# MaaniGhaffari/cvo-rgbd

Measured on AMD Instinct MI355X. Metric: frame-pair registrations/sec, higher is better.
Workload: dtype f32; 1 GPU; BASELINE configs[1] shape: 64 distinct synthetic 10000x10000 RGB-D cloud pairs (xyz + 5-dim colour) per align_many call, cvo align() to convergence, clouds resident in HBM; points_fixed=10000, points_moving=10000, mode=cvo, batch=64

## Files before the change

### cvo-rgbd_amd/csrc/cvo_capi.cpp

```cpp
#include "cvo_internal.h"

using namespace cvo_dev;
using namespace cvo_impl;

namespace cvo_impl {

int fail(cvo_hip_ctx *ctx, int code, const char *msg)
{
    if (ctx) ctx->err = msg;
    return code;
}

static std::atomic<bool> g_engine_debug{false};
bool engine_debug_on() { return g_engine_debug.load(std::memory_order_relaxed); }

namespace {
struct OptDef {
    const char *key;
    const char *env;
    int env_kind;
    double env_value;
};
const OptDef kOptions[] = {
    {"graph_capture", "CVO_HIP_GRAPH", 1, 1.0},           {"no_graph", "CVO_HIP_NO_GRAPH", 1, 1.0},
    {"head_graphs", "CVO_HIP_RUN_GRAPHS", 1, 1.0},        {"head_mode", "CVO_HIP_NO_HEAD", 1, 0.0},
    {"resident_runs", "CVO_HIP_NO_RUN", 1, 0.0},          {"run_solvers_max", "CVO_HIP_RUN_G_MAX", 2, 0.0},
    {"run_candidates_max", "CVO_HIP_RUN_CAND", 2, 0.0},   {"run_timeout_ms", nullptr, 0, 0.0},
    {"run_fault", nullptr, 0, 0.0},                       {"merged_launches", "CVO_HIP_NO_MERGE", 1, 0.0},
    {"async_builds", "CVO_HIP_NO_ASYNC", 1, 0.0},         {"list_pass_blocks", "CVO_HIP_PROC_BLOCKS", 2, 0.0},
    {"post_debug", "CVO_HIP_POST_DEBUG", 1, 1.0},         {"mailbox_timeout_s", "CVO_HIP_MAILBOX_TIMEOUT_S", 2, 0.0},
    {"candidate_records", "CVO_HIP_NO_CAND", 1, 0.0},     {"sync_upload", "CVO_HIP_SYNC_UPLOAD", 1, 1.0},
    {"engine_debug", "CVO_HIP_ENGINE_DEBUG", 1, 1.0},     {"one_launch_hand_over", "CVO_HIP_NO_CLOUD_ONE", 1, 0.0},
    {"small_calls_alone", "CVO_HIP_NO_ALONE", 1, 0.0},    {"fused_groups", "CVO_HIP_NO_FUSE", 1, 0.0},
    {"engines", "CVO_HIP_ENGINES_FORCE", 2, 0.0},         {"list_init", "CVO_HIP_LIST_INIT", 2, 0.0},
    {"kept_pack", "CVO_HIP_NO_PACK", 1, 0.0},             {"list_margin", "CVO_HIP_LIST_MARGIN", 2, 0.0},
    {"final_mirror", "CVO_HIP_NO_FINAL_MIRROR", 1, 0.0},  {"twist_on_shared_gpu", "CVO_HIP_TWIST_ON_SHARED_GPU", 1, 1.0},
    {"comm_debug", "CVO_HIP_COMM_DEBUG", 1, 1.0},         {"wait_policy", "CVO_HIP_WAIT_POLICY", 2, 0.0},
    {"acvo_runs", "CVO_HIP_NO_ACVO_RUN", 1, 0.0},         {"tail_alone", "CVO_HIP_TAIL_ALONE", 2, 0.0},         {"side_builds", "CVO_HIP_SIDE", 1, 1.0},
    {"run_build_at", "CVO_HIP_RUN_BUILD_AT", 2, 0.0},         {"alone_max", "CVO_HIP_ALONE_MAX", 2, 0.0},
    {"narrow_merge", "CVO_HIP_NARROW_MERGE", 1, 1.0},     {"narrow_blocks", "CVO_HIP_NARROW_BLOCKS", 2, 0.0},
    {"engine_crowd", "CVO_HIP_ENGINE_CROWD", 2, 0.0},     {"engine_merge_max", "CVO_HIP_ENGINE_MERGE_MAX", 2, 0.0},
    {"matches_combine", nullptr, 0, 0.0},                 {"scan_chunk", nullptr, 0, 0.0},
    {"record_narrow", "CVO_HIP_NO_RECORD_NARROW", 1, 0.0}, {"list_stale_max", "CVO_HIP_LIST_STALE_MAX", 2, 0.0},
};
void env_defaults(cvo_hip_ctx *ctx)
{
    for (const OptDef &d : kOptions) {
        if (!d.env) continue;
        const char *e = getenv(d.env);
        if (!e) continue;
        (void)apply_option(ctx, d.key, d.env_kind == 1 ? d.env_value : atof(e));
    }
}
}

int apply_option(cvo_hip_ctx *ctx, const char *key, double v)
{
    auto is = [&](const char *k) { return std::strcmp(key, k) == 0; };
    const bool on = v != 0.0;
    CtxOptions &o = ctx->opt;
    if (is("graph_capture")) { ctx->use_graphs = on && !o.no_graph; if (!ctx->use_graphs) drop_graphs(ctx); }
    else if (is("no_graph")) { o.no_graph = on; if (on) { ctx->use_graphs = false; drop_graphs(ctx); } }
    else if (is("head_graphs")) ctx->head_graphs = on;
    else if (is("head_mode")) ctx->allow_head = on;
    else if (is("resident_runs")) ctx->allow_run = on;
    else if (is("run_solvers_max")) {
        int cus = 0;
        if (hipDeviceGetAttribute(&cus, hipDeviceAttributeMultiprocessorCount, ctx->device) != hipSuccess || cus <= 0) cus = RUN_G + 8;
        ctx->run_g_max = v > 0.0 ? std::max(8, std::min((int)RUN_G, (int)v)) : std::max(8, std::min((int)RUN_G, cus - 8));
    }
    else if (is("run_candidates_max")) { if (v < 0.0) return CVO_HIP_ERR_INVALID; o.run_cand = (int)v; }
    else if (is("run_timeout_ms")) { if (v < 0.0 || v > 6.0e4) return CVO_HIP_ERR_INVALID; o.run_timeout_ms = v; }
    else if (is("run_fault")) { if (v < 0.0) return CVO_HIP_ERR_INVALID; o.run_fault = (int)v; }
    else if (is("merged_launches")) ctx->allow_merge = on;
    else if (is("async_builds")) ctx->allow_async = ctx->allow_async_self = on;
    else if (is("list_pass_blocks")) {
        const int b = (int)v;
        if (b == 0) { ctx->proc_blocks_forced = false; ctx->proc_blocks = ctx->proc_blocks_default = PROC_BLOCKS; }
        else if (b == 64 || b == 128 || b == 256 || b == 512 || b == 1024) { ctx->proc_blocks = ctx->proc_blocks_default = b; ctx->proc_blocks_forced = true; }
        else return CVO_HIP_ERR_INVALID;
    }
    else if (is("post_debug")) o.post_debug = on;
    else if (is("mailbox_timeout_s")) { if (!(v > 0.0)) return CVO_HIP_ERR_INVALID; o.mailbox_timeout_s = v; }
    else if (is("candidate_records")) o.no_cand = !on;
    else if (is("sync_upload")) o.sync_upload = on;
    else if (is("engine_debug")) { o.engine_debug = on; if (on) g_engine_debug.store(true, std::memory_order_relaxed); }
    else if (is("one_launch_hand_over")) o.no_cloud_one = !on;
    else if (is("small_calls_alone")) o.no_alone = !on;
    else if (is("fused_groups")) o.no_fuse = !on;
    else if (is("engines")) { if (v < 0.0 || v > 8.0) return CVO_HIP_ERR_INVALID; o.engines_force = (int)v; }
    else if (is("list_init")) { if (v < 0.0) return CVO_HIP_ERR_INVALID; o.list_init = v; }
    else if (is("kept_pack")) o.no_pack = !on;
    else if (is("matches_combine")) o.matches_combine = on;
    else if (is("scan_chunk")) { if (v < 0.0 || v > (double)SCAN_CHUNK) return CVO_HIP_ERR_INVALID; o.scan_chunk = (int)v; }
    else if (is("list_margin")) { if (v > 4.0) return CVO_HIP_ERR_INVALID; o.list_margin = v < 0.0 ? -1.0f : (float)v; }
    else if (is("record_narrow")) o.record_narrow = on;
    else if (is("list_stale_max")) { if (!(v >= 1.0 && v <= 64.0)) return CVO_HIP_ERR_INVALID; o.list_stale_max = (float)v; }
    else if (is("final_mirror")) o.no_final_mirror = !on;
    else if (is("twist_on_shared_gpu")) o.twist_on_shared_gpu = on;
    else if (is("comm_debug")) o.comm_debug = on;
    else if (is("wait_policy")) { if (v < 0.0 || v > 2.0) return CVO_HIP_ERR_INVALID; o.wait_policy = (int)v; }
    else if (is("acvo_runs")) o.no_acvo_run = !on;
    else if (is("tail_alone")) { if (v < 0.0 || v > 32.0) return CVO_HIP_ERR_INVALID; o.tail_alone = (int)v; }
    else if (is("run_restart")) o.no_restart = !on;
    else if (is("side_builds")) o.no_side_builds = !on;
    else if (is("run_build_at")) { if (!(v > 0.0 && v <= 1.0)) return CVO_HIP_ERR_INVALID; o.run_build_at = (float)v; }
    else if (is("alone_max")) { if (v < 0.0 || v > 64.0) return CVO_HIP_ERR_INVALID; o.alone_max = (int)v; }
    else if (is("narrow_merge")) o.narrow_merge = on;
    else if (is("narrow_blocks")) { const int b = (int)v; if (b != 0 && b != 32 && b != 64) return CVO_HIP_ERR_INVALID; o.narrow_blocks = b; }
    else if (is("engine_crowd")) { if (v < 0.0) return CVO_HIP_ERR_INVALID; o.engine_crowd = (int)std::min(v, 1.0e6); }
    else if (is("engine_merge_max")) { if (v < 0.0 || v > 32.0) return CVO_HIP_ERR_INVALID; o.engine_merge_max = (int)v; }
    else return CVO_HIP_ERR_INVALID;
    return CVO_HIP_OK;
}

const char *params_problem(const cvo_hip_params &p)
{
    if (p.mode != CVO_HIP_MODE_CVO && p.mode != CVO_HIP_MODE_ACVO)
        return "params.mode must be CVO_HIP_MODE_CVO or CVO_HIP_MODE_ACVO (MATLAB: default_params() returns mode CVO)";
    if (p.max_iter < 0) return "params.max_iter < 0";
    const float pos[] = {p.ell_init, p.sigma, p.sp_thres, p.c, p.d, p.c_ell, p.c_sigma};
    const char *pos_name[] = {"ell_init", "sigma", "sp_thres", "c", "d", "c_ell", "c_sigma"};
    static thread_local char msg[96];
    for (int i = 0; i < 7; ++i)
        if (!(pos[i] > 0.0f) || !std::isfinite(pos[i])) {
            snprintf(msg, sizeof(msg), "params.%s must be positive and finite", pos_name[i]);
            return msg;
        }
    if (p.mode == CVO_HIP_MODE_ACVO && (!(p.c_sp_thres > 0.0f) || !std::isfinite(p.c_sp_thres)))
        return "params.c_sp_thres must be positive and finite";
    if (p.mode == CVO_HIP_MODE_ACVO && (!(p.ell_max_init > 0.0f) || !std::isfinite(p.ell_max_init) ||
                                        !(p.ell_min >= 0.0f) || !std::isfinite(p.dl_step)))
        return "params.ell_max_init / ell_min / dl_step out of range";
    const float fin[] = {p.min_step, p.eps, p.eps_2, p.color_scale, p.ell_min};
    for (float v : fin)
        if (!std::isfinite(v)) return "params: min_step, eps, eps_2, color_scale, ell_min must be finite";
    if (p.color_scale < 0.0f) return "params.color_scale < 0";
    return nullptr;
}

DevParams make_dev_params(const cvo_hip_params &p)
{
    DevParams d{};
    d.mode = p.mode;
    d.max_iter = p.max_iter;
    d.ell_init = p.ell_init;
    d.ell_min = p.ell_min;
    d.ell_max_init = p.ell_max_init;
    d.sp = p.sp_thres;
    d.c_sp = (p.mode == CVO_HIP_MODE_ACVO) ? p.c_sp_thres : p.sp_thres;
// ... 146 lines not shown
    static_assert(sizeof(DevState) >= 2048 + sizeof(DevHead), "the mirrors share a pinned DevState");
    ctx->run_mirror = ctx->done_mirror + 32;
    ctx->hint_mirror = ctx->done_mirror + 48;
    ctx->side_mirror = ctx->done_mirror + 64;
    *ctx->side_mirror = 0;
    *ctx->done_mirror = 0;
    *ctx->progress_mirror = 0;
    *ctx->run_mirror = 0;
    *ctx->hint_mirror = -1;
    {
        int cus = 0;
        if (hipDeviceGetAttribute(&cus, hipDeviceAttributeMultiprocessorCount, device) != hipSuccess || cus <= 0) cus = RUN_G + 8;
        ctx->run_g_max = std::max(8, std::min((int)RUN_G, cus - 8));
    }
    ctx->use_graphs = ctx->own_stream;
    env_defaults(ctx);
    if (ctx->opt.post_debug) {
        if (hipMalloc((void **)&ctx->post_dbg, 8 * sizeof(long long)) != hipSuccess) return bail(CVO_HIP_ERR_NOMEM);
        (void)hipMemset(ctx->post_dbg, 0, 8 * sizeof(long long));
    }
    *out = ctx;
    return CVO_HIP_OK;
}

int cvo_hip_destroy(cvo_hip_ctx *ctx)
{
    cvo_lock::Api api_guard;
    if (!ctx) return CVO_HIP_OK;
    (void)hipSetDevice(ctx->device);
    if (ctx->stream) (void)hipStreamSynchronize(ctx->stream);
    for (auto &ev : ctx->events) { (void)hipEventDestroy(ev.a); (void)hipEventDestroy(ev.b); }
    for (int i = 0; i < kPollSlots; ++i)
        if (ctx->poll_ev[i]) (void)hipEventDestroy(ctx->poll_ev[i]);
    if (ctx->comm) cvo_comm_destroy(ctx->comm);
    for (void *q : ctx->mail_opened)
        if (q) (void)hipIpcCloseMemHandle(q);
    if (ctx->comm_table) (void)hipFree(ctx->comm_table);
    if (ctx->mailbox) (void)hipFree(ctx->mailbox);
    drop_graphs(ctx);
    ctx->table.destroy();
    if (ctx->post_dbg) {
        long long h[8];
        if (hipMemcpy(h, ctx->post_dbg, sizeof(h), hipMemcpyDeviceToHost) == hipSuccess && h[0] > 0)
            fprintf(stderr, "[cvo_hip] post-step part over %lld launches, avg ticks: state load %.0f, reduce %.0f, "
                    "cubic %.0f, exp+update %.0f, prepare %.0f; head mode: block 0 of the flow launch start to end %.0f\n",
                    h[0], (double)h[1] / h[0], (double)h[2] / h[0],
                    (double)h[3] / h[0], (double)h[4] / h[0], (double)h[5] / h[0], (double)h[7] / h[0]);
        (void)hipFree(ctx->post_dbg);
    }
    for (void *p : {(void *)ctx->fixed.pos, (void *)ctx->fixed.feat, (void *)ctx->moving.pos,
                    (void *)ctx->moving.feat, (void *)ctx->fixed.seg, (void *)ctx->moving.seg,
                    (void *)ctx->scratch_a.pos, (void *)ctx->scratch_a.feat, (void *)ctx->scratch_a.seg,
                    (void *)ctx->scratch_b.pos, (void *)ctx->scratch_b.feat, (void *)ctx->scratch_b.seg, (void *)ctx->st, (void *)ctx->st2, ctx->part_flow.p, ctx->part_xx.p,
                    ctx->part_yy.p, ctx->part_step.p, ctx->part_hess.p, ctx->part_score.p, ctx->part_matches.p, ctx->run_mail.p, (void *)ctx->trace_dev, ctx->kept_cnt.p, ctx->pos_bt.p, ctx->cand[0].p, ctx->cand[1].p, ctx->cand[2].p, ctx->cand_xyb.p, ctx->cand_cnt_xyb.p, ctx->cand_sfb[0].p, ctx->cand_sfb[1].p, ctx->cand_cnt_sfb[0].p, ctx->cand_cnt_sfb[1].p, ctx->cand_cnt[0].p,
                    ctx->cand_cnt[1].p, ctx->cand_cnt[2].p})
        if (p) (void)hipFree(p);
    for (int l = 0; l < LIST_N; ++l) {
        if (ctx->lists[l].a.p) (void)hipFree(ctx->lists[l].a.p);
        if (ctx->lists[l].b.p) (void)hipFree(ctx->lists[l].b.p);
    }
    if (ctx->st_host) (void)hipHostFree(ctx->st_host);
    if (ctx->score_pin) (void)hipHostFree(ctx->score_pin);
    if (ctx->match_stage.p) (void)hipHostFree(ctx->match_stage.p);
    if (ctx->scan_stage.p) (void)hipHostFree(ctx->scan_stage.p);
    if (ctx->scan_dev.p) (void)hipFree(ctx->scan_dev.p);
    for (Cloud *c : {&ctx->fixed, &ctx->moving, &ctx->scratch_a, &ctx->scratch_b}) {
        if (c->pending && (c->wait_ev || c->ready_ev)) (void)hipEventSynchronize(c->wait_ev ? c->wait_ev : c->ready_ev);
        if (c->stage) (void)hipHostFree(c->stage);
        if (c->bbox_pin) (void)hipHostFree(c->bbox_pin);
        if (c->ready_ev) (void)hipEventDestroy(c->ready_ev);
    }
    for (DevBuf *b : {&ctx->raw_xyz, &ctx->raw_feat, &ctx->sort_keys[0], &ctx->sort_keys[1], &ctx->sort_idx[0],
                      &ctx->sort_idx[1], &ctx->sort_tmp})
        if (b->p) (void)hipFree(b->p);
    if (ctx->bbox_dev) (void)hipFree(ctx->bbox_dev);
    if (ctx->bbox_host) (void)hipHostFree(ctx->bbox_host);
    if (ctx->side_stream) { (void)hipStreamSynchronize(ctx->side_stream); (void)hipStreamDestroy(ctx->side_stream); }
    if (ctx->own_stream && ctx->stream) (void)hipStreamDestroy(ctx->stream);
    delete ctx;
    return CVO_HIP_OK;
}

int cvo_hip_set_params(cvo_hip_ctx *ctx, const cvo_hip_params *p)
{
    cvo_lock::Api api_guard;
    if (!ctx || !p) return CVO_HIP_ERR_INVALID;
    if (const char *why = params_problem(*p)) return fail(ctx, CVO_HIP_ERR_INVALID, why);
    drop_graphs(ctx);
    ctx->prm = *p;
    ctx->dprm = make_dev_params(*p);
    for (Cloud *c : {&ctx->fixed, &ctx->moving, &ctx->scratch_a, &ctx->scratch_b}) c->self.valid = false;
    return CVO_HIP_OK;
}

int cvo_hip_shard_range(int n, int rank, int world, int *lo, int *hi)
{
    if (!lo || !hi || world <= 0 || rank < 0 || rank >= world || n < 0) return CVO_HIP_ERR_INVALID;
    *lo = (int)((int64_t)n * rank / world);
    *hi = (int)((int64_t)n * (rank + 1) / world);
    return CVO_HIP_OK;
}

int cvo_hip_set_shard(cvo_hip_ctx *ctx, int row_lo, int row_hi, int srow_lo, int srow_hi)
{
    cvo_lock::Api api_guard;
    if (!ctx || row_lo < 0 || row_hi < row_lo || srow_lo < 0 || srow_hi < srow_lo)
        return CVO_HIP_ERR_INVALID;
// ... 169 lines not shown
    h->kc_ell = -1.0f;
    rc = fill_filter_geometry(ctx, h);
    if (rc) return rc;
    compute_filter_bounds(h, false);
    rc = push_state_fields(ctx, offsetof(DevState, kc),
                           offsetof(DevState, xi) - offsetof(DevState, kc));
    if (rc) return rc;
    for (bool redo = true; redo;) {
        rc = zero_counters(ctx);
        if (!rc) rc = enqueue_flow(ctx, true, 0, false, nullptr, 0);
        if (!rc) rc = check_overflow_and_grow(ctx, &redo);
        if (rc) return rc;
        if (multi_rank(ctx)) {
            double nnz = 0.0;
            rc = fetch_red(ctx, RED_FLOW + 8, 1, &nnz);
            if (rc) return rc;
            if (nnz != nnz) redo = true;
        }
    }
    rc = fetch_red(ctx, RED_FLOW, 13, out13);
    if (!rc && ctx->profiling) rc = drain_events(ctx);
    return rc;
}

int cvo_hip_step_coeffs(cvo_hip_ctx *ctx, const float omega[3], const float v[3], float ell,
                        double bcde[4])
{
    cvo_lock::Api api_guard;
    if (!ctx || !omega || !v || !bcde) return CVO_HIP_ERR_INVALID;
    HIP_TRY(ctx, hipSetDevice(ctx->device));
    if (!ctx->have_tf) return fail(ctx, CVO_HIP_ERR_INVALID, "transform_pcd not called");
    int rc = mailboxes_usable(ctx);
    if (rc) return rc;
    DevState *h = &ctx->st_host[kPollSlots];
    h->kc = make_kconsts(ctx->dprm, ell);
    h->kc_ell = -1.0f;
    rc = fill_filter_geometry(ctx, h);
    if (rc) return rc;
    compute_filter_bounds(h, false);
    h->xi = cvo_math::make_xi_consts(omega, v);
    rc = push_state_fields(ctx, offsetof(DevState, kc),
                           offsetof(DevState, omega) - offsetof(DevState, kc));
    if (rc) return rc;
    int rlo, rhi, slo, shi;
    shard_ranges(ctx, rlo, rhi, slo, shi);
    for (bool redo = true; redo;) {
        rc = zero_counters(ctx);
        if (!rc) rc = enqueue_filter(ctx, LIST_XY, ctx->fixed, rlo, rhi, 0, ctx->moving, 1, 0);
        if (!rc) rc = enqueue_process(ctx, PROC_FLOW, LIST_XY, ctx->part_flow, ctx->fixed.pos,
                                      ctx->fixed.feat, 0, ctx->moving.pos, ctx->moving.feat, 1, 0, 0);
        if (!rc) rc = check_overflow_and_grow(ctx, &redo);
        if (rc) return rc;
    }
    rc = enqueue_step(ctx, 0, false, nullptr, 0);
    if (rc) return rc;
    rc = fetch_red(ctx, RED_STEP, 4, bcde);
    if (!rc && ctx->profiling) rc = drain_events(ctx);
    return rc;
}

int cvo_hip_pick_step(const double bcde[4], float min_step, float *step)
{
    if (!bcde || !step) return CVO_HIP_ERR_INVALID;
    *step = cvo_math::pick_step(bcde, min_step);
    return CVO_HIP_OK;
}

int cvo_hip_exp_se3(const float omega[3], const float v[3], float dt, float dR[9], float dT[3])
{
    if (!omega || !v || !dR || !dT) return CVO_HIP_ERR_INVALID;
    cvo_math::exp_se3(omega, v, dt, dR, dT);
    return CVO_HIP_OK;
}

int cvo_hip_dist_se3(const float omega[3], const float v[3], float dt, float *dist)
{
    if (!omega || !v || !dist) return CVO_HIP_ERR_INVALID;
    *dist = cvo_math::dist_se3(omega, v, dt);
    return CVO_HIP_OK;
}

int cvo_hip_function_inner_product(cvo_hip_ctx *ctx, float ell, float *out)
{
    cvo_lock::Api api_guard;
    if (!ctx || !out) return CVO_HIP_ERR_INVALID;
    HIP_TRY(ctx, hipSetDevice(ctx->device));
    DevParams dp = ctx->dprm;
    dp.log_sp_s2 = (float)std::log((double)(ctx->prm.sp_thres / ctx->prm.sigma / ctx->prm.sigma));
    if (ctx->prm.mode == CVO_HIP_MODE_ACVO) {
        dp.c_sp = ctx->prm.sp_thres;
        dp.tau_c = (float)(-2.0 * ctx->prm.c_ell * ctx->prm.c_ell *
                           (double)(float)std::log((double)(dp.c_sp / ctx->prm.c_sigma / ctx->prm.c_sigma)));
    }
    int rc = mailboxes_usable(ctx);
    if (rc) return rc;
    DevState *h = &ctx->st_host[kPollSlots];
    h->kc = make_kconsts(dp, ell);
    h->kc_ell = -1.0f;
    rc = fill_filter_geometry(ctx, h);
    if (rc) return rc;
    compute_filter_bounds(h, true);
    h->done = 0;
    rc = push_state_fields(ctx, offsetof(DevState, kc),
                           offsetof(DevState, xi) - offsetof(DevState, kc));
    if (rc) return rc;
    rc = push_state_fields(ctx, offsetof(DevState, done), sizeof(int32_t));
    if (rc) return rc;
// ... 120 lines not shown
        hipMemcpy(clk, reinterpret_cast<const char *>(ctx->st) + offsetof(DevState, run_clk), sizeof(clk), hipMemcpyDeviceToHost) != hipSuccess)
        return CVO_HIP_ERR_HIP;
    for (int q = 0; q < 16; ++q) clocks16[q] = clk[q];
    return CVO_HIP_OK;
}

int cvo_hip_set_option(cvo_hip_ctx *ctx, const char *key, double value)
{
    cvo_lock::Api api_guard;
    if (!ctx || !key) return CVO_HIP_ERR_INVALID;
    if (hipSetDevice(ctx->device) != hipSuccess) return CVO_HIP_ERR_HIP;
    const int rc = apply_option(ctx, key, value);
    if (rc) return fail(ctx, rc, "cvo_hip_set_option: unknown key or value out of range");
    return CVO_HIP_OK;
}

int cvo_hip_get_option(const cvo_hip_ctx *ctx, const char *key, double *value)
{
    if (!ctx || !key || !value) return CVO_HIP_ERR_INVALID;
    auto is = [&](const char *k) { return std::strcmp(key, k) == 0; };
    const CtxOptions &o = ctx->opt;
    if (is("graph_capture")) *value = ctx->use_graphs;
    else if (is("no_graph")) *value = o.no_graph;
    else if (is("head_graphs")) *value = ctx->head_graphs;
    else if (is("head_mode")) *value = ctx->allow_head;
    else if (is("resident_runs")) *value = ctx->allow_run;
    else if (is("run_solvers_max")) *value = ctx->run_g_max;
    else if (is("run_candidates_max")) *value = o.run_cand;
    else if (is("run_timeout_ms")) *value = o.run_timeout_ms;
    else if (is("run_fault")) *value = o.run_fault;
    else if (is("merged_launches")) *value = ctx->allow_merge;
    else if (is("async_builds")) *value = ctx->allow_async;
    else if (is("list_pass_blocks")) *value = ctx->proc_blocks_forced ? ctx->proc_blocks : 0;
    else if (is("post_debug")) *value = o.post_debug;
    else if (is("mailbox_timeout_s")) *value = o.mailbox_timeout_s;
    else if (is("candidate_records")) *value = !o.no_cand;
    else if (is("sync_upload")) *value = o.sync_upload;
    else if (is("engine_debug")) *value = o.engine_debug;
    else if (is("one_launch_hand_over")) *value = !o.no_cloud_one;
    else if (is("small_calls_alone")) *value = !o.no_alone;
    else if (is("fused_groups")) *value = !o.no_fuse;
    else if (is("engines")) *value = o.engines_force;
    else if (is("narrow_merge")) *value = o.narrow_merge;
    else if (is("narrow_blocks")) *value = o.narrow_blocks;
    else if (is("engine_crowd")) *value = o.engine_crowd;
    else if (is("engine_merge_max")) *value = o.engine_merge_max;
    else if (is("list_init")) *value = o.list_init;
    else if (is("kept_pack")) *value = !o.no_pack;
    else if (is("matches_combine")) *value = o.matches_combine;
    else if (is("scan_chunk")) *value = o.scan_chunk;
    else if (is("list_margin")) *value = o.list_margin;
    else if (is("record_narrow")) *value = o.record_narrow;
    else if (is("list_stale_max")) *value = o.list_stale_max;
    else if (is("final_mirror")) *value = !o.no_final_mirror;
    else if (is("twist_on_shared_gpu")) *value = o.twist_on_shared_gpu;
    else if (is("comm_debug")) *value = o.comm_debug;
    else if (is("wait_policy")) *value = o.wait_policy;
    else if (is("acvo_runs")) *value = !o.no_acvo_run;
    else if (is("tail_alone")) *value = o.tail_alone;
    else if (is("tail_handovers")) *value = (double)ctx->tail_handovers;
    else if (is("run_restart")) *value = !o.no_restart;
    else if (is("side_builds")) *value = !o.no_side_builds;
    else if (is("run_build_at")) *value = o.run_build_at;
    else if (is("side_builds_launched")) *value = (double)ctx->side_builds_launched;
    else if (is("alone_max")) *value = o.alone_max;
    else if (is("run_timeouts")) *value = (double)ctx->run_timeouts;
    else if (is("list_grows")) *value = (double)ctx->list_grows;
    else if (is("async_builds_named")) *value = (double)ctx->async_stats[0];
    else if (is("async_stalls")) *value = (double)ctx->async_stats[1];
    else if (is("run_aborts")) *value = (double)ctx->run_aborts;
    else if (is("no_run_backoff")) *value = ctx->no_run_backoff;
    else return CVO_HIP_ERR_INVALID;
    return CVO_HIP_OK;
}

long long cvo_hip_get_mirror_retries(void) { return mirror_retries().load(std::memory_order_relaxed); }

int cvo_hip_synchronize(cvo_hip_ctx *ctx)
{
    cvo_lock::Api api_guard;
    if (!ctx) return CVO_HIP_ERR_INVALID;
    HIP_TRY(ctx, hipStreamSynchronize(ctx->stream));
    return CVO_HIP_OK;
}


}
```

### cvo-rgbd_amd/csrc/cvo_device.h

```cpp
#pragma once

#include <hip/hip_runtime.h>
#include <hip/hip_ext.h>
#include <stddef.h>
#include <stdint.h>

#include "cvo_hip.h"
#include "se3_math.hpp"

namespace cvo_dev {

constexpr int FEAT_STRIDE = 8;
constexpr int FEAT_INDEX_SLOT = 5;

constexpr int BLOCK = 256;
constexpr int TILES_PER_WAVE = 4;
constexpr int ROWS_PER_WAVE = 16 * TILES_PER_WAVE;
constexpr int ROWS_PER_TILE = 4 * ROWS_PER_WAVE;
constexpr float PAD_BIG = 1.0e30f;
constexpr int PROC_BLOCKS = 1024;
constexpr int PROC_WAVES = PROC_BLOCKS * 4;

constexpr int NSUB = 256;
constexpr int PROC_PARTS = PROC_BLOCKS / NSUB;
// ... 62 lines not shown
    unsigned long long p[RUN_GEN][RUN_CHAINS][2 * RUN_NV];
    unsigned long long entry_ticket;
    unsigned long long entry_go;
    unsigned long long side_done;
    unsigned long long side_req;
};
constexpr int RUN_G_SIDE = 128;

struct KernConsts {
    float tau;
    float tau_c;
    float sp;
    float inv_c;
    float inv_d;
    float inv_l3;
    float cb, cg, cd;
    float cscale;
    double s2_d;
    double cs2_d;
    double ninv_2l2;
    double ninv_2cl2;
};

struct DevParams {
    int32_t mode, max_iter;
    float ell_init, ell_min, ell_max_init;
    float sp, c_sp;
    float c, d, c_ell;
    float min_step, eps, eps_2;
    float log_sp_s2;
    float tau_c;
    float list_margin;
    int32_t async_xy;
    float build_at;
    int32_t async_self;
    float color_scale;
    float run_cand_cap;
    int32_t record_narrow;
    float list_stale_max;
    double s2_d, cs2_d, dl_step;
};

struct alignas(16) DevHead {
    float R[9], T[3];
    float ell, ell_max;
    float Rt[9], t[3];
    float used_Rt[9], used_t[3];
    KernConsts kc;
    float kc_ell, kc_pad_;
    float center[3];
    float xmax, y0max;
    float tauf[3];
    int32_t n_fixed;
    uint32_t pad0_;
    float list_r[3];
    int32_t list_ok[3];
    int32_t reuse[3];
    int32_t ck_nblk[3];
    float list_Rt[9], list_t[3];
    float rec_r;
    int32_t narrow;
    float rec_Rt[9], rec_t[3];
    int32_t list_stat[3];
    int32_t async_stat[2];
    int32_t rec_pad_;
    int32_t xy_active, xy_target, stall, xy_fresh;
    int32_t xy_ok[2];
    int32_t xy_ck[2];
    float xy_r[2];
    float tauf_build;
    float r_last;
    float xy_Rt[2][9], xy_t[2][3];
    int32_t sf_active[2], sf_target[2], sf_fresh[2];
    int32_t sf_ok[2][2];
    int32_t sf_ck[2][2];
    float sf_r[2][2];
    float sf_tauf_build[2];
    cvo_math::XiConsts xi;
    float omega[3], v[3];
    double dl;
    double red[RED_N];
    int32_t k;
    int32_t done;
    int32_t iter;
    int32_t n_exec;
    int32_t n_slots;
    int32_t pending;
    unsigned long long mail_snap;
    int32_t run_hint;
    int32_t head_check_;
    int32_t rec_count[2];
};
enum { REC_NARROW = 1, REC_BOUNDED = 2 };
CVO_HD unsigned head_check_mix(unsigned x, unsigned y, unsigned z, unsigned w, unsigned piece)
{
    return (x * 0x9E3779B1u + y * 0x85EBCA77u + z * 0xC2B2AE3Du + w * 0x27D4EB2Fu) ^ (piece * 0x165667B1u + 0x9E3779B9u);
}
struct DevState : DevHead {
    uint32_t sub[LIST_N][NSUB];
    uint32_t ovf[2][8];
    uint32_t built[3][64];
    int32_t run_count;
    int32_t run_entered;
    int32_t run_iterations;
    int32_t run_candidates;
    int32_t run_last_entered, run_last_aborted;
    long long run_clk[16];
    unsigned long long mail_seq;
    unsigned long long run_seq;
};
static_assert(LIST_N <= 8, "DevState::ovf holds 8 lists");
constexpr size_t DEVSTATE_INIT_BYTES = offsetof(DevState, mail_seq);
constexpr size_t DEVSTATE_HEAD_BYTES = sizeof(DevHead);
static_assert(offsetof(DevState, sub) == sizeof(DevHead) && sizeof(DevHead) % 16 == 0, "the tail follows the head");

constexpr int MAXG = 16;
template <class A> struct Grp { A a[MAXG]; };
constexpr int ENGINE_SLOTS = 32;
// ... 8 lines not shown
    TileEntry *tiles;
    TileEntry *tiles_b;
    int async_xy;
    uint32_t subcap;
    int list;
    int row_lo, row_hi;
    int nb;
    int jt;
    int tf_a, tf_b;
    int check_done;
    int gx, gy;
    long long *dbg;
    float4 *pos_bt;
};

struct ProcessArgs {
    const float4 *pos_a;
    const float *feat_a;
    const float4 *pos_b;
    const float *feat_b;
    const TileEntry *tiles;
    const TileEntry *tiles_b;
    int async_xy;
    int async_self;
    uint2 *kept_ij;
    float *kept_a;
    uint32_t *kept_cnt;
    double *partials;
    DevState *st;
    DevState *st2;
    uint32_t subcap;
    uint32_t kept_wcap;
    int nblk;
    const double *flow_part;
    const double *xx_part;
    const double *yy_part;
    cvo_hip_trace *trace; int trace_cap;
    int acvo;
    int32_t *done_mirror;
    int list;
    int row_hi, nb;
    int first_counted;
    int tf_a, tf_b;
    int check_done;
    int weight;
    uint2 *cand;
    uint32_t *cand_cnt;
    uint2 *cand_b;
    uint32_t *cand_cnt_b;
    int need_d2;
    const CommTable *comm;
    int kept_packed;
    unsigned kept_ebase;
};

enum { POST_REDUCE = 1, POST_MATH = 2 };

struct PostFlowArgs {
    DevState *st;
    const double *part_flow;
    const double *part_xx;
    const double *part_yy;
    cvo_hip_trace *trace; int trace_cap;
    int flags;
    int check_done;
    int32_t *done_mirror;
    int nblk;
    const CommTable *comm;
    DevParams prm;
};

struct PostStepArgs {
    DevState *st;
    DevState *st2;
    const double *part_step;
    cvo_hip_trace *trace; int trace_cap;
    int flags;
    int check_done;
    long long *dbg;
    int32_t *done_mirror;
    int ck_nblk[3];
    int32_t *progress_mirror;
    int nblk;
    const CommTable *comm;
    DevHead *final_mirror;
    uint32_t *build_mask;
    uint32_t slot_bit;
    RunMail *run_mail;
    int32_t *run_mirror;
    int32_t *hint_mirror;
    int run_iters;
    int run_g_max;
    long long run_timeout_ticks;
    int32_t *side_mirror;
    float run_build_at;
    int run_fault;
    DevParams prm;
};

constexpr size_t kTableHeaderBytes = 256;
constexpr int MAX_OPS = 10;
struct OpArgs {
    ProcessArgs p;
    FilterArgs f;
    union {
        PostFlowArgs pf;
        PostStepArgs ps;
    };
    int np, n0, n1, n2;
};
struct Slot {
    int active;
    int pad_[3];
    OpArgs op[MAX_OPS];
};

CVO_HD KernConsts make_kconsts(const DevParams &p, float ell)
{
    KernConsts k;
    const float l = ell;
    k.tau = (float)(-2.0 * l * l * (double)p.log_sp_s2);
    k.tau_c = p.tau_c;
    k.sp = p.sp;
// ... 604 lines not shown
```

### cvo-rgbd_amd/csrc/cvo_internal.h

```cpp
#pragma once
#include "cvo_hip.h"

#include <hip/hip_runtime.h>

#include <algorithm>
#include <atomic>
#include <chrono>
#include <cmath>
#include <cstddef>
#include <cstdint>
#include <cstdio>
#include <cstdlib>
#include <cstring>
#include <deque>
#include <memory>
#include <mutex>
#include <new>
#include <string>
#include <thread>
#include <vector>

#include "cvo_cloud.h"
#include "cvo_comm.h"
#include "cvo_device.h"
// ... 119 lines not shown
            st[z] = image[(size_t)z];
        }
        if (hipMemcpyAsync(&dev[lo], &st[lo], n * sizeof(Slot), hipMemcpyHostToDevice, s) != hipSuccess) return -1;
        if (arm(s) != 0) return -1;
        if (hipEventRecord(stage_ev[b], s) != hipSuccess) return -1;
        stage_used[b] = true;
        return 0;
    }
};

struct PlanGraph {
    std::vector<TLaunch> pre;
    std::vector<TLaunch> plan;
    int iterations = 0;
    hipGraph_t graph = nullptr;
    hipGraphExec_t exec = nullptr;
    uint64_t stamp = 0;
};
struct PlanCache {
    std::vector<PlanGraph> graphs;
    uint64_t clock = 0;
    long long hits = 0, captures = 0;
    int fails = 0;
    void drop()
    {
        for (auto &g : graphs) {
            if (g.exec) (void)hipGraphExecDestroy(g.exec);
            if (g.graph) (void)hipGraphDestroy(g.graph);
        }
        graphs.clear();
    }
};
constexpr int kPollSlots = 4;
constexpr int kEvProcFlow = 10, kEvProcStep = 11;
constexpr int kProcStepTwist = 100;
constexpr int kFlowBuild = 101;
constexpr int kFilterAhead = 102;

struct RecOp {
    enum Kind { FILTER, PROCESS, POST_FLOW, POST_STEP } kind;
    int mode = 0;
    FilterArgs f{};
    ProcessArgs p{};
    PostFlowArgs pf{};
    PostStepArgs ps{};
};


}

using namespace cvo_dev;
using namespace cvo_impl;

struct CtxOptions {
    bool no_cand = false;
    bool no_graph = false;
    bool sync_upload = false;
    bool engine_debug = false;
    bool no_cloud_one = false;
    bool no_alone = false;
    bool no_fuse = false;
    bool no_pack = false;
    bool matches_combine = true;
    int scan_chunk = 0;
    bool no_final_mirror = false;
    bool twist_on_shared_gpu = false;
    bool comm_debug = false;
    bool post_debug = false;
    bool no_side_builds = true;
    float run_build_at = 0.6f;
    bool no_restart = false;
    bool no_acvo_run = false;
    int tail_alone = 8;
    int alone_max = 0;
    int engines_force = 0;
    int narrow_blocks = 0;
    bool narrow_merge = false;
    int engine_crowd = 2;
    int engine_merge_max = 2;
    double list_init = 0.0;
    float list_margin = -1.0f;
    bool record_narrow = true;
    float list_stale_max = 3.0f;
    int run_cand = 0;
    double mailbox_timeout_s = 5.0;
    double run_timeout_ms = 0.0;
    int run_fault = 0;
    int wait_policy = 0;
};

struct cvo_hip_ctx {
    CtxOptions opt;
    int no_run_backoff = 0;
    long long side_builds_launched = 0;
    long long tail_handovers = 0;
    long long run_aborts = 0;
    int list_stats[3] = {0, 0, 0};
    int async_stats[2] = {0, 0};
    long long list_grows = 0;
    long long run_timeouts = 0;
    int device = 0;
    hipStream_t stream = nullptr;
    bool own_stream = false;
    cvo_hip_params prm{};
    DevParams dprm{};
    Cloud fixed, moving;
    Cloud scratch_a, scratch_b;
    DevState *st = nullptr;
    DevHead *st2 = nullptr;
    bool head_mode = false;
    bool allow_head = true;
    DevState *st_host = nullptr;
    int32_t *done_mirror = nullptr;
    int32_t *progress_mirror = nullptr;
    DevHead *final_mirror = nullptr;
    int32_t *run_mirror = nullptr;
    int32_t *hint_mirror = nullptr;
    int32_t *side_mirror = nullptr;
    hipStream_t side_stream = nullptr;
    std::vector<TLaunch> plan_side;
    DevBuf run_mail;
    bool plan_has_final_mirror = false;
    bool allow_run = true;
    int run_g_max = RUN_G;
    int run_g_call = RUN_G;
    bool call_no_spec = false;
    int big_run_backoff = 0;
    bool spec_first_run = true;
    bool head_graphs = false;
    int run_small_max = 0;
    int run_nnz_max = 0;
    std::vector<TLaunch> plan_pre;
    std::vector<RecOp> *rec = nullptr;
    int proc_blocks = PROC_BLOCKS;
    int proc_blocks_default = PROC_BLOCKS;
    bool proc_blocks_forced = false;
    DevBuf raw_xyz, raw_feat;
    DevBuf sort_keys[2], sort_idx[2], sort_tmp;
    float *bbox_dev = nullptr;
    float *bbox_host = nullptr;
    FilterArgs xy_build{};
    bool have_xy_build = false;
    bool allow_async = true;
    bool crowded = false;
    DevBuf cand[3], cand_cnt[3];
    DevBuf cand_xyb, cand_cnt_xyb;
    DevBuf cand_sfb[2], cand_cnt_sfb[2];
    int ck_nblk[3] = {0, 0, 0};
    DevBuf pos_bt;
    bool lone = true;
    bool allow_async_self = true;
    bool use_async_self = false;
    bool use_async = false;
    bool in_loop = false;
    bool plan_recording = false;
    bool merge_twist = false;
    bool allow_merge = true;
    cvo_hip_trace *cur_trace = nullptr;
    int cur_trace_cap = 0;
    hipEvent_t poll_ev[kPollSlots]{};
    DevBuf part_flow, part_xx, part_yy, part_step;
    DevBuf part_hess;
    DevBuf part_score;
    struct ScorePin *score_pin = nullptr;
    DevBuf part_matches;
    PinBuf match_stage;
    DevBuf scan_dev;
    PinBuf scan_stage;
    List lists[LIST_N];
    DevBuf kept_cnt;
    cvo_hip_trace *trace_dev = nullptr;
    int trace_dev_cap = 0;
    bool have_tf = false;
    int row_lo = 0, row_hi = -1, srow_lo = 0, srow_hi = -1;
    bool sharded = false;
    cvo_comm *comm = nullptr;
    Mailbox *mailbox = nullptr;
    CommTable *comm_table = nullptr;
    void *mail_opened[MAX_WORLD] = {};
    int mail_rank = 0, mail_world = 0;
    bool mail_shared_device = false;
    unsigned long long mail_dev_id = 0;
    bool mail_broken = false;
    cvo_hip_allreduce_fn user_allreduce = nullptr;
    void *user_allreduce_arg = nullptr;
    bool profiling = false;
    long long *post_dbg = nullptr;
    TableBuf table;
    PlanCache plans;
    std::vector<TLaunch> plan;
    hipStream_t loop_stream = nullptr;
    bool warm = false;
    bool use_graphs = true;
    int iter_tag = -1;
    std::vector<EventPair> events;
    cvo_hip_profile prof{};
    std::string err;
};

namespace cvo_impl {

// ... 12 lines not shown
    cvo_hip_trace *trace = nullptr;
    int trace_cap = 0;
    int *n_iter = nullptr;
    int enq = 0;
    int batches = 0;
    int checked = 0;
    int executed_base = 0;
    int phase = 0;
    int rc = CVO_HIP_OK;
    bool in_group = false;
    int runs_enq = 0;
    bool run_waiting = false;
    bool spec_pending = false;
    bool paced_nb = false;
    int idle_seen = 0;
    int side_seen = 0;
    int side_launched = 0;
    int restarts = 0;
    bool paced = false;
};

int fail(cvo_hip_ctx *ctx, int code, const char *msg);
bool engine_debug_on();
int apply_option(cvo_hip_ctx *ctx, const char *key, double value);
inline bool runs_allowed(const cvo_hip_ctx *ctx) { return ctx->allow_run && ctx->no_run_backoff <= 0; }
const char *params_problem(const cvo_hip_params &p);
DevParams make_dev_params(const cvo_hip_params &p);
int cloud_ready(cvo_hip_ctx *ctx, Cloud &c);
int cloud_reserve(cvo_hip_ctx *ctx, Cloud &c, const float *xyz, const float *feat, int n, int layout);
int upload_cloud(cvo_hip_ctx *ctx, Cloud &c, const float *xyz, const float *feat, int n, int layout, bool on_device = false);
FilterPlan plan_filter(int nrows, int nb);
int ensure_buf(cvo_hip_ctx *ctx, DevBuf &b, size_t bytes);
int ensure_list(cvo_hip_ctx *ctx, int list, int nrows, int nb, double at_least);
void shard_ranges(const cvo_hip_ctx *ctx, int &rlo, int &rhi, int &slo, int &shi);
int fill_filter_geometry(cvo_hip_ctx *ctx, DevState *h);
int mailboxes_usable(cvo_hip_ctx *ctx);
bool host_reduce(const cvo_hip_ctx *ctx);
bool multi_rank(const cvo_hip_ctx *ctx);
DevParams loop_params(const cvo_hip_ctx *ctx);
hipStream_t loop_stream(const cvo_hip_ctx *ctx);
int enqueue_filter(cvo_hip_ctx *ctx, int list, const Cloud &ca, int row_lo, int row_hi, int tf_a, const Cloud &cb, int tf_b, int check_done);
int kept_format(const cvo_hip_ctx *ctx, unsigned *ebase);
KeptView kept_view(const cvo_hip_ctx *ctx);
int enqueue_process(cvo_hip_ctx *ctx, int mode, int list, DevBuf &part, const float4 *pos_a, const float *feat_a, int tf_a,
                    const float4 *pos_b, const float *feat_b, int tf_b, int first_counted, int check_done);
int drain_events(cvo_hip_ctx *ctx, int n_exec = -1, const DevState *fin = nullptr);
int reduce_over_ranks(cvo_hip_ctx *ctx, int off, int count);
int enqueue_flow(cvo_hip_ctx *ctx, bool tf_moving, int check_done, bool do_math, cvo_hip_trace *trace, int trace_cap);
int enqueue_step(cvo_hip_ctx *ctx, int check_done, bool do_math, cvo_hip_trace *trace, int trace_cap);
int check_overflow_and_grow(cvo_hip_ctx *ctx, bool *redo);
int prepare_buffers(cvo_hip_ctx *ctx);
int enqueue_iterations(cvo_hip_ctx *ctx, int count, int tag0, int trace_cap);
void drop_graphs(cvo_hip_ctx *ctx);
TLaunch mk_launch(int kernel, int q, unsigned gx, unsigned gz, unsigned smem = 0);
bool plan_lone(const std::vector<RecOp> &ops, Slot &slot, std::vector<TLaunch> &plan, const bool allow_head, bool *head_mode,
               std::vector<TLaunch> *pre = nullptr, std::vector<TLaunch> *side = nullptr);
void set_build_masks(Slot &slot, const std::vector<TLaunch> &plan, uint32_t *masks, int z);
bool plan_fused(const std::vector<const std::vector<RecOp> *> &ops, const std::vector<Slot *> &slots, int zdim, std::vector<TLaunch> &plan);
int run_plan(const Slot *tab, PlanCache &cache, const std::vector<TLaunch> &plan, hipStream_t s, bool use_graph, int iterations,
             const std::vector<TLaunch> *pre = nullptr);
int record_iteration(cvo_hip_ctx *ctx, std::vector<RecOp> &ops, int trace_cap);
int prepare_lone_plan(cvo_hip_ctx *ctx, int trace_cap);
int launch_batch(cvo_hip_ctx *ctx, int tag0, int trace_cap, bool with_run = false, int slots = kBatch, bool small_run = false, bool two_runs = false);
constexpr int kNoRunBackoff = 64;
constexpr int kBigRunBackoff = 16;
constexpr int kShortBatch = 2;
constexpr int kRunBatchSlots = 2;
int zero_counters(cvo_hip_ctx *ctx);
int push_state_fields(cvo_hip_ctx *ctx, size_t off, size_t bytes);
int push_pose_fields(cvo_hip_ctx *ctx, const DevHead *img, bool with_consts);
int enqueue_flow_reduce(cvo_hip_ctx *ctx, const CommTable *comm);
int fetch_red(cvo_hip_ctx *ctx, int off, int count, double *out);
void decide_scheme(cvo_hip_ctx *ctx);
std::atomic<long long> &mirror_retries();
int job_begin(AlignJob &j);
int job_finish(AlignJob &j);
int job_continue_alone(AlignJob &j);
int job_pump(AlignJob &j, bool block);

}
```

### cvo-rgbd_amd/csrc/cvo_job.cpp

```cpp
#include "cvo_internal.h"

using namespace cvo_dev;
using namespace cvo_impl;

namespace cvo_impl {

void decide_scheme(cvo_hip_ctx *ctx)
{
    const bool small_pair = (double)ctx->fixed.n * (double)ctx->moving.n <= 2.5e7;
    if (!ctx->proc_blocks_forced)
        ctx->proc_blocks = ctx->proc_blocks_default = small_pair ? PROC_BLOCKS / 2 : PROC_BLOCKS;
    ctx->use_async = ctx->allow_async && !ctx->crowded && !ctx->profiling && !multi_rank(ctx) &&
                     !(ctx->prm.color_scale > 0.0f) &&
                     (double)ctx->fixed.n * (double)ctx->moving.n <= 2.0e8;
    ctx->use_async_self = ctx->use_async && ctx->allow_async_self && ctx->lone &&
                          ctx->prm.mode == CVO_HIP_MODE_ACVO;
    const double npairs = (double)ctx->fixed.n * (double)ctx->moving.n;
    if (ctx->use_async_self && !ctx->proc_blocks_forced)
        ctx->proc_blocks = ctx->proc_blocks_default = npairs <= 6.0e7 ? PROC_BLOCKS / 8 : PROC_BLOCKS / 4;
    if (!ctx->proc_blocks_forced && !ctx->use_async_self && ctx->use_async && ctx->lone && ctx->allow_head &&
        ctx->prm.mode == CVO_HIP_MODE_CVO)
    {
        const bool runs = runs_allowed(ctx) && ctx->fixed.np <= 65536 && ctx->moving.np <= 65536;
        ctx->proc_blocks = ctx->proc_blocks_default =
// ... 110 lines not shown
    decide_scheme(ctx);
    hipStream_t s = loop_stream(ctx);
    HIP_TRY(ctx, hipMemsetAsync(reinterpret_cast<char *>(ctx->st) + offsetof(DevState, n_slots), 0, sizeof(int32_t), s));
    HIP_TRY(ctx, hipMemsetAsync(reinterpret_cast<char *>(ctx->st) + offsetof(DevState, run_count), 0, 4 * sizeof(int32_t), s));
    HIP_TRY(ctx, hipMemsetAsync(reinterpret_cast<char *>(ctx->st) + offsetof(DevState, run_last_entered), 0, 2 * sizeof(int32_t), s));
    launch_prepare(ctx->st, loop_params(ctx), s, ctx->table.raw ? ctx->table.masks() : nullptr);
    HIP_TRY(ctx, hipGetLastError());
    const int prc = prepare_buffers(ctx);
    if (prc) return prc;
    ctx->head_mode = false;
    const int rc = prepare_lone_plan(ctx, 0);
    if (rc) return rc;
    j.enq = j.batches = j.checked = 0;
    j.runs_enq = 0;
    j.run_waiting = false;
    j.spec_pending = false;
    j.side_seen = 0;
    j.side_launched = 0;
    const int g_call = std::max(8, std::min(ctx->run_g_max, ctx->run_g_call));
    ctx->run_nnz_max = g_call * RUN_BLOCK * (RUN_R + RUN_L);
    ctx->run_small_max = 3 * RUN_G_SMALL * RUN_BLOCK;
    if (ctx->prm.mode == CVO_HIP_MODE_ACVO) {
        ctx->run_nnz_max = (int)(0.8 * g_call * RUN_BLOCK * RUN_A);
        ctx->run_small_max = (int)(0.8 * 2 * RUN_G_SMALL * RUN_BLOCK);
    }
    if (ctx->opt.run_cand > 0) ctx->run_nnz_max = ctx->opt.run_cand;
    j.phase = 0;
    ++ctx->tail_handovers;
    return CVO_HIP_OK;
}

int job_finish(AlignJob &j)
{
    cvo_hip_ctx *ctx = j.ctx;
    cvo_hip_state *s = j.s;
    const DevState &f = ctx->st_host[0];
    ctx->have_tf = false;
    if (f.done == DONE_COMM_ERROR) {
        ctx->mail_broken = true;
        if (ctx->opt.comm_debug)
            fprintf(stderr, "[cvo_hip] rank %d of %d: exchange timed out at iteration k = %d (executed %d), mail_seq %llu, mail_snap %llu, slots %d, twist in launch %d\n",
                    ctx->mail_rank, ctx->mail_world, f.k, f.n_exec, (unsigned long long)f.mail_seq, (unsigned long long)f.mail_snap, f.n_slots,
                    (int)(ctx->plan.size() == 4));
        return fail(ctx, CVO_HIP_ERR_COMM, "mailbox all-reduce timed out: a peer rank never delivered its partial sums "
                                           "(the mailboxes must be created and connected again on every rank)");
    }
    if (f.done == DONE_RUN_TIMEOUT)
        return fail(ctx, CVO_HIP_ERR_RUN, "a resident run timed out and the registration could not be redone without runs");
    if (f.done == RUNNING || f.done == NEED_BIGGER_LIST)
        return fail(ctx, CVO_HIP_ERR_INVALID, "align loop ended without a verdict");
    const int executed = f.n_exec;
    for (int q = 0; q < 3; ++q) ctx->list_stats[q] = f.list_stat[q];
    for (int q = 0; q < 2; ++q) ctx->async_stats[q] = f.async_stat[q];
    if (j.trace_cap > 0 && executed > 0)
        HIP_TRY(ctx, hipMemcpy(j.trace, ctx->trace_dev,
                               (size_t)std::min(executed, j.trace_cap) * sizeof(cvo_hip_trace),
                               hipMemcpyDeviceToHost));
    if (executed > 0) cvo_math::tf_to_mat4(f.used_Rt, f.used_t, s->transform);
    std::memcpy(s->R, f.R, sizeof(s->R));
    std::memcpy(s->T, f.T, sizeof(s->T));
    s->ell = f.ell;
    s->ell_max = f.ell_max;
    s->iter = f.iter;
    std::memcpy(s->prev_transform, s->transform, sizeof(s->transform));
    cvo_math::mat4_mul(s->accum_transform, s->transform, s->accum_transform);
    float Rt[9], t[3];
    cvo_math::inverse_tf(s->R, s->T, Rt, t);
    cvo_math::tf_to_mat4(Rt, t, s->transform);
    if (j.n_iter) *j.n_iter = executed;
    if (ctx->profiling) return drain_events(ctx, executed, &f);
    return CVO_HIP_OK;
}

int job_pump(AlignJob &j, bool block)
{
    cvo_hip_ctx *ctx = j.ctx;
    if (j.phase == 2) return 1;
    auto finish_with = [&](int rc) { j.rc = rc; j.phase = 2; return 1; };
    if (hipSetDevice(ctx->device) != hipSuccess) return finish_with(CVO_HIP_ERR_HIP);
    if (j.phase == 0 && (block || j.paced_nb) && (j.paced || j.paced_nb) && !host_reduce(ctx) && !ctx->profiling) {
        const int limit = (ctx->use_async ? 3 : 1) * ctx->prm.max_iter + 4 * kBatch;
        unsigned spins = 0;
        int idle_seen = 0;
        const auto t_enter = std::chrono::steady_clock::now();
        for (;;) {
            if (*(volatile int32_t *)ctx->done_mirror != RUNNING) break;
            const int runs_word = *(volatile int32_t *)ctx->run_mirror;
            const int runs = runs_word & (RUN_MIRROR_ABORTED - 1);
            const int slots = *(volatile int32_t *)ctx->progress_mirror;
            if (!ctx->plan_side.empty()) {
                const int want = *(volatile int32_t *)ctx->side_mirror;
                if (want != 0 && want != j.side_seen) {
                    j.side_seen = want;
                    for (const TLaunch &l : ctx->plan_side) launch_table(ctx->table.dev, l, ctx->side_stream);
                    if (hipGetLastError() != hipSuccess) return finish_with(fail(ctx, CVO_HIP_ERR_HIP, "launching a side build failed"));
                    ++j.side_launched;
                    ++ctx->side_builds_launched;
                }
            }
            const int lead = ctx->head_mode ? 2 : 0;
            bool go;
            if (j.run_waiting) {
                go = runs >= j.runs_enq;
                if (go) {
                    if (runs_word & RUN_MIRROR_ABORTED) { ctx->big_run_backoff = kBigRunBackoff; ++ctx->run_aborts; }
                    else if (j.spec_pending) ctx->spec_first_run = (runs_word & RUN_MIRROR_ENTERED) != 0;
// ... 216 lines not shown
```

### cvo-rgbd_amd/csrc/cvo_kernels.hip

```cpp
#include <algorithm>
#include <atomic>
#include <cstdlib>

#include "cvo_device.h"
#include "cvo_pair.h"

namespace cvo_dev {

typedef float f32x4 __attribute__((ext_vector_type(4)));

__device__ __forceinline__ float mv_row(const float *m, float x, float y, float z)
{
    return (m[0] * x + m[1] * y) + m[2] * z;
}

constexpr int FILTER_KMAX = 64;
size_t filter_smem_bytes(int jt)
{
    return (size_t)jt * 16 + ROWS_PER_TILE * 16 + 4 * TILE_STAGE * sizeof(TileEntry) +
           FILTER_KMAX * 4 * 4;
}

__device__ __forceinline__ void flush_tiles(const TileEntry *stage, int n, int lane, unsigned rot, unsigned region,
                                            const FilterArgs &a, int list, TileEntry *tiles, const int par)
{
    static_assert(TILE_STAGE <= 128, "two entries per lane");
    constexpr int sh = DEAL_SHIFT, L = 1 << sh;
    unsigned base = 0;
    if (lane < 32) {
        int cnt = 0;
        for (int c = (int)(((unsigned)lane - rot) & 31u); (c << sh) < n; c += 32) cnt += min(n - (c << sh), L);
        if (cnt) base = atomicAdd(&a.st->sub[list][((unsigned)lane << 3) | region], (unsigned)cnt);
    }
    bool over = false;
#pragma unroll
    for (int h = 0; h < 2; ++h) {
        const int k = lane + 64 * h;
        const unsigned c = (unsigned)k >> sh;
        const unsigned j = (c + rot) & 31u;
        const unsigned pos = (unsigned)__shfl((int)base, (int)j, 64) + ((c >> 5) << sh) + ((unsigned)k & (unsigned)(L - 1));
        if (k < n) {
            if (pos < a.subcap) tiles[(size_t)((j << 3) | region) * a.subcap + pos] = stage[k];
            else over = true;
        }
    }
    if (__ballot(over) != 0ull && lane == 0)
        atomicOr(&a.st->ovf[par][list], 1u);
}

__device__ __forceinline__ void pretransform_body(const FilterArgs &a, const unsigned bid, const unsigned nblocks)
{
    if (!a.pos_bt) return;
    if (a.check_done && a.st->done != 0) return;
    const float *Rt = a.st->Rt;
    const float *tt = a.st->t;
    for (unsigned j = bid * BLOCK + threadIdx.x; j < (unsigned)a.nb; j += nblocks * BLOCK) {
        const float4 y0 = a.pos_b[j];
        float4 y = apply_tf(Rt, tt, y0);
        y.w = y0.w;
        a.pos_bt[j] = y;
    }
}

template <bool PIPE = true>
__device__ __forceinline__ void filter_body(const FilterArgs &a, const unsigned bid, const unsigned nblocks,
                                            const DevState *__restrict__ hd, const int par)
{
// ... 226 lines not shown
    const long long want = std::min<long long>(per_region * 8, std::max<long long>(cap, 8));
    return (unsigned)((want + 7) / 8 * 8);
}

void launch_filter(const FilterArgs &a, dim3 grid, hipStream_t s, hipEvent_t ev_start,
                   hipEvent_t ev_stop)
{
    Grp<FilterArgs> g;
    g.a[0] = a;
    g.a[0].gx = (int)grid.x; g.a[0].gy = (int)grid.y;
    grid = dim3(filter_grid_x((long long)grid.x * grid.y, filter_blocks_max()), 1, 1);
    if (ev_start && ev_stop)
        hipExtLaunchKernelGGL(k_filter, grid, dim3(BLOCK), filter_smem_bytes(a.jt), s, ev_start,
                              ev_stop, 0, g);
    else
        hipLaunchKernelGGL(k_filter, grid, dim3(BLOCK), filter_smem_bytes(a.jt), s, g);
}

void launch_filter_group(const FilterArgs *a, int n, hipStream_t s)
{
    Grp<FilterArgs> g;
    dim3 grid(1, 1, (unsigned)n);
    int jt = 0;
    const long long cap = std::max<long long>(64, filter_blocks_max() / (2 * n));
    for (int i = 0; i < n; ++i) {
        g.a[i] = a[i];
        grid.x = std::max(grid.x, filter_grid_x((long long)a[i].gx * a[i].gy, cap));
        jt = std::max(jt, a[i].jt);
    }
    hipLaunchKernelGGL(k_filter, grid, dim3(BLOCK), filter_smem_bytes(jt), s, g);
}


__device__ __forceinline__ float colour_weight(const KernConsts &kc, const float4 fa0, const float fa4,
                                               const float4 fb0, const float fb4, const double *etab)
{
    const float d2c = d2_feat(fa0, fa4, fb0, fb4);
    if (!(d2c < kc.tau_c)) return 0.0f;
    return (float)(kc.cs2_d * exp_neg((double)d2c * kc.ninv_2cl2, etab));
}
__device__ __forceinline__ float weight_from_ck(const KernConsts &kc, float d2, float ck, const double *etab)
{
    const float k = (float)(kc.s2_d * exp_neg((double)d2 * kc.ninv_2l2, etab));
    const float a = ck * k;
    return a > kc.sp ? a : 0.0f;
}


template <int MODE> struct NAcc;
template <> struct NAcc<PROC_FLOW> { static constexpr int n = NACC_FLOW; };
template <> struct NAcc<PROC_STEP> { static constexpr int n = NACC_STEP; };
template <> struct NAcc<PROC_SELF> { static constexpr int n = NACC_SELF; };

__device__ __forceinline__ double div6(double x)
{
    const double c = 0x1.5555555555555p-3;
    const double q0 = x * c;
    const double r = __builtin_fma(-6.0, q0, x);
    return __builtin_fma(r, c, q0);
}

__device__ __forceinline__ uint2 list_load(const uint2 *p)
{
#ifdef CVO_NT_LISTS
    typedef unsigned u32x2 __attribute__((ext_vector_type(2)));
    const u32x2 v = __builtin_nontemporal_load(reinterpret_cast<const u32x2 *>(p));
    return make_uint2(v.x, v.y);
#else
    return *p;
#endif
}

__device__ __forceinline__ const float4 *gather16(const void *base, unsigned byte_off)
{
    return reinterpret_cast<const float4 *>(static_cast<const char *>(base) + byte_off);
}

struct ProcHead {
    const float *Rt, *tt;
    const cvo_math::XiConsts *xi;
    KernConsts kc;
    int done_word;
    int n_fixed;
    int second;
    unsigned list_bad;
    int ck_nblk;
    int par;
    uint2 *cand;
    uint32_t *cand_cnt;
    int need_d2;
    int narrow;
    float rec_lim;
};

template <int MODE>
__device__ __forceinline__ ProcHead proc_head_global(const ProcessArgs &a, const DevState *st, const int par)
{
    ProcHead h;
    h.Rt = st->Rt; h.tt = st->t; h.xi = &st->xi;
    h.kc = st->kc;
    h.done_word = a.check_done ? (st->done | (a.async_xy ? st->stall : 0)) : 0;
    h.n_fixed = (MODE == PROC_SELF && a.first_counted) ? st->n_fixed : 0;
    h.second = ((MODE == PROC_FLOW && a.async_xy && st->xy_active == 1) ||
                (MODE == PROC_SELF && a.async_self && st->sf_active[a.async_self - 1] == 1)) ? 1 : 0;
    const bool ahead = (MODE == PROC_FLOW && a.async_xy) || (MODE == PROC_SELF && a.async_self);
    h.list_bad = ahead ? 0u : a.st->ovf[par][MODE == PROC_STEP ? (int)LIST_KEPT : a.list];
    h.ck_nblk = st->ck_nblk[a.list];
    h.par = par;
    h.cand = a.cand; h.cand_cnt = a.cand_cnt;
    h.need_d2 = a.need_d2;
    h.narrow = (MODE == PROC_FLOW && !a.async_xy) ? st->narrow : 0;
    h.rec_lim = (h.narrow & REC_BOUNDED) ? st->rec_r * st->rec_r : PAD_BIG;
    return h;
}


struct PairSrc {
    const CVO_GLOBAL char *pos_a; const float *feat_a;
    const CVO_GLOBAL char *pos_b; const float *feat_b;
    int tf_a, tf_b;
};
#ifdef CVO_NO_PIN
constexpr bool kPinBuild = false;
#else
constexpr bool kPinBuild = true;
#endif
#ifdef CVO_NO_PF
constexpr bool kPrefetchBuild = false;
#else
constexpr bool kPrefetchBuild = true;
#endif
template <bool PIN, class T> __device__ __forceinline__ const CVO_GLOBAL char *pin_global(const T *p)
{
    unsigned long long v = (unsigned long long)p;
    if (PIN && kPinBuild) asm volatile("" : "+s"(v));
    return (const CVO_GLOBAL char *)v;
}
template <bool PIN> __device__ __forceinline__ unsigned pin_u32(unsigned v)
{
    if (PIN && kPinBuild) asm volatile("" : "+s"(v));
    return v;
}
template <bool PIN> __device__ __forceinline__ PairSrc pin_pair_src(const ProcessArgs &a)
{
    PairSrc p;
    p.pos_a = pin_global<PIN>(a.pos_a); p.pos_b = pin_global<PIN>(a.pos_b);
    p.feat_a = a.feat_a; p.feat_b = a.feat_b;
    p.tf_a = (int)pin_u32<PIN>((unsigned)a.tf_a); p.tf_b = (int)pin_u32<PIN>((unsigned)a.tf_b);
    return p;
}
__device__ __forceinline__ void store8(const CVO_GLOBAL char *base, unsigned idx, unsigned x, unsigned y)
{
    u32x2_t v; v.x = x; v.y = y;
    CVO_GLOBAL u32x2_t *q = reinterpret_cast<CVO_GLOBAL u32x2_t *>(const_cast<CVO_GLOBAL char *>(base)) + idx;
#ifdef CVO_NT_KEPT_ST
    __builtin_nontemporal_store(v, q);
#else
    *q = v;
#endif
}

__device__ __forceinline__ cvo_math::XiConsts xi_uniform(const cvo_math::XiConsts &g)
{
    cvo_math::XiConsts xc;
    auto uni = [](float x) { return __int_as_float(__builtin_amdgcn_readfirstlane(__float_as_int(x))); };
#pragma unroll
    for (int q = 0; q < 3; ++q) {
        xc.omega[q] = uni(g.omega[q]); xc.v[q] = uni(g.v[q]);
        xc.u2[q] = uni(g.u2[q]); xc.u3[q] = uni(g.u3[q]); xc.u4[q] = uni(g.u4[q]);
    }
#pragma unroll
    for (int q = 0; q < 9; ++q) {
        xc.W2[q] = uni(g.W2[q]); xc.W3[q] = uni(g.W3[q]); xc.W4[q] = uni(g.W4[q]);
    }
    return xc;
}

__device__ __forceinline__ void pair_flow_sums(const KernConsts &kc, const float4 xi, const float4 yj, const float w, const float d2,
                                           const int need_d2, double *acc)
{
    const float c0 = xi.y * yj.z - xi.z * yj.y;
    const float c1 = xi.z * yj.x - xi.x * yj.z;
    const float c2 = xi.x * yj.y - xi.y * yj.x;
    const float f0 = yj.x - xi.x, f1 = yj.y - xi.y, f2 = yj.z - xi.z;
    const float ac = kc.inv_c * w, ad = kc.inv_d * w;
    acc[0] += (double)(ac * c0);
    acc[1] += (double)(ac * c1);
    acc[2] += (double)(ac * c2);
    acc[3] += (double)(ad * f0);
    acc[4] += (double)(ad * f1);
    acc[5] += (double)(ad * f2);
#ifdef CVO_SUM_A_ALWAYS
    acc[6] += (double)w;
    if (need_d2) acc[7] += (double)((kc.inv_l3 * w) * d2);
#else
    if (need_d2) {
        acc[6] += (double)w;
        acc[7] += (double)((kc.inv_l3 * w) * d2);
    }
#endif
}

__device__ __forceinline__ void step_tail(const float w, const float beta, const float gamma, const float delta, const float epsil, double *acc)
{
    const double A = (double)w;
    const double b = (double)beta, g = (double)gamma;
    acc[0] += (double)(w * beta);
#ifdef CVO_STEP_TAIL_LITERAL
    acc[1] += A * (g + (double)(beta * beta) / 2.0);
    acc[2] += A * ((double)(delta + beta * gamma) + div6((double)(beta * beta * beta)));
    acc[3] += A * ((((double)(epsil + beta * delta) + 0.5 * b * b * g) + 0.5 * g * g) +
                   1 / 24.0 * b * b * b * b);
#else
    acc[1] = __builtin_fma(A, __builtin_fma((double)(beta * beta), 0.5, g), acc[1]);
    acc[2] = __builtin_fma(A, __builtin_fma((double)(beta * beta * beta), 0x1.5555555555555p-3,
                                            (double)(delta + beta * gamma)), acc[2]);
    const double b2 = b * b, hg = 0.5 * g;
    double t = __builtin_fma(b2, hg, (double)(epsil + beta * delta));
    t = __builtin_fma(hg, g, t);
    t = __builtin_fma(b2 * (1 / 24.0), b2, t);
    acc[3] = __builtin_fma(A, t, acc[3]);
#endif
}

__device__ __forceinline__ void pair_step_sums(const KernConsts &kc, const cvo_math::XiConsts &xc, const float4 yj, const float e0,
                                           const float e1, const float e2, const float w, double *acc)
{
    float xiz[3], xi2z[3], xi3z[3], xi4z[3];
    xiz[0] = (xc.omega[1] * yj.z - xc.omega[2] * yj.y) + xc.v[0];
    xiz[1] = (xc.omega[2] * yj.x - xc.omega[0] * yj.z) + xc.v[1];
    xiz[2] = (xc.omega[0] * yj.y - xc.omega[1] * yj.x) + xc.v[2];
#pragma unroll
    for (int r = 0; r < 3; ++r) {
        xi2z[r] = mv_row(xc.W2 + 3 * r, yj.x, yj.y, yj.z) + xc.u2[r];
        xi3z[r] = mv_row(xc.W3 + 3 * r, yj.x, yj.y, yj.z) + xc.u3[r];
        xi4z[r] = mv_row(xc.W4 + 3 * r, yj.x, yj.y, yj.z) + xc.u4[r];
    }
    const float normxiz2 = (xiz[0] * xiz[0] + xiz[1] * xiz[1]) + xiz[2] * xiz[2];
    const float xz12 = -((xiz[0] * xi2z[0] + xiz[1] * xi2z[1]) + xiz[2] * xi2z[2]);
    const float eps_c = ((xi2z[0] * xi2z[0] + xi2z[1] * xi2z[1]) + xi2z[2] * xi2z[2]) +
                        2 * ((xiz[0] * xi3z[0] + xiz[1] * xi3z[1]) + xiz[2] * xi3z[2]);
    const float cb = kc.cb, cg = kc.cg, cd = kc.cd;
    const float beta = ((cb * xiz[0]) * e0 + (cb * xiz[1]) * e1) + (cb * xiz[2]) * e2;
    const float g_dot = ((2.0f * xi2z[0]) * e0 + (2.0f * xi2z[1]) * e1) + (2.0f * xi2z[2]) * e2;
    const float gamma = cg * (normxiz2 + g_dot);
    const float d_dot = ((-xi3z[0]) * e0 + (-xi3z[1]) * e1) + (-xi3z[2]) * e2;
    const float delta = cd * (xz12 + d_dot);
    const float e_dot = ((2.0f * xi4z[0]) * e0 + (2.0f * xi4z[1]) * e1) + (2.0f * xi4z[2]) * e2;
    const float epsil = cg * (eps_c + e_dot);
    step_tail(w, beta, gamma, delta, epsil, acc);
}

typedef float f32x2 __attribute__((ext_vector_type(2)));
__device__ __forceinline__ void pair_step_sums2(const KernConsts &kc, const cvo_math::XiConsts &xc, const f32x2 yx, const f32x2 yy, const f32x2 yz,
                                                const f32x2 e0, const f32x2 e1, const f32x2 e2, const f32x2 w, double *acc)
{
    f32x2 xiz[3], xi2z[3], xi3z[3], xi4z[3];
    xiz[0] = (xc.omega[1] * yz - xc.omega[2] * yy) + xc.v[0];
    xiz[1] = (xc.omega[2] * yx - xc.omega[0] * yz) + xc.v[1];
    xiz[2] = (xc.omega[0] * yy - xc.omega[1] * yx) + xc.v[2];
#pragma unroll
    for (int r = 0; r < 3; ++r) {
        xi2z[r] = ((xc.W2[3 * r] * yx + xc.W2[3 * r + 1] * yy) + xc.W2[3 * r + 2] * yz) + xc.u2[r];
        xi3z[r] = ((xc.W3[3 * r] * yx + xc.W3[3 * r + 1] * yy) + xc.W3[3 * r + 2] * yz) + xc.u3[r];
        xi4z[r] = ((xc.W4[3 * r] * yx + xc.W4[3 * r + 1] * yy) + xc.W4[3 * r + 2] * yz) + xc.u4[r];
    }
    const f32x2 normxiz2 = (xiz[0] * xiz[0] + xiz[1] * xiz[1]) + xiz[2] * xiz[2];
    const f32x2 xz12 = -((xiz[0] * xi2z[0] + xiz[1] * xi2z[1]) + xiz[2] * xi2z[2]);
    const f32x2 eps_c = ((xi2z[0] * xi2z[0] + xi2z[1] * xi2z[1]) + xi2z[2] * xi2z[2]) +
                        2.0f * ((xiz[0] * xi3z[0] + xiz[1] * xi3z[1]) + xiz[2] * xi3z[2]);
    const float cb = kc.cb, cg = kc.cg, cd = kc.cd;
    const f32x2 beta = ((cb * xiz[0]) * e0 + (cb * xiz[1]) * e1) + (cb * xiz[2]) * e2;
    const f32x2 g_dot = ((2.0f * xi2z[0]) * e0 + (2.0f * xi2z[1]) * e1) + (2.0f * xi2z[2]) * e2;
    const f32x2 gamma = cg * (normxiz2 + g_dot);
    const f32x2 d_dot = ((-xi3z[0]) * e0 + (-xi3z[1]) * e1) + (-xi3z[2]) * e2;
    const f32x2 delta = cd * (xz12 + d_dot);
    const f32x2 e_dot = ((2.0f * xi4z[0]) * e0 + (2.0f * xi4z[1]) * e1) + (2.0f * xi4z[2]) * e2;
    const f32x2 epsil = cg * (eps_c + e_dot);
    step_tail(w.x, beta.x, gamma.x, delta.x, epsil.x, acc);
    step_tail(w.y, beta.y, gamma.y, delta.y, epsil.y, acc);
}

template <int MODE, int WEIGHT = 0, int CK = 0, class ARGS = ProcessArgs>
__device__ __forceinline__ float eval_pair(const ARGS &a, const ProcHead &hd, const KernConsts &kc, unsigned i,
                                           unsigned j, float w, double *acc,
                                           const cvo_math::XiConsts &xc, const double *etab = nullptr,
                                           const int first_counted = 0, float *ck_io = nullptr,
                                           uint2 *pf_out = nullptr, const CVO_GLOBAL char *pf_base = nullptr, unsigned pf_idx = 0,
                                           float *d2_out = nullptr )
{
    const float *Rt = hd.Rt;
    const float *tt = hd.tt;
    constexpr bool need_w = MODE != PROC_STEP && CK != 2;
    float4 xi = load_pos<need_w>(a.pos_a, i * 16u);
    float4 yj = load_pos<need_w>(a.pos_b, j * 16u);
    if (pf_out) *pf_out = load8(pf_base, pf_idx);
    float4 fa0 = make_float4(0.f, 0.f, 0.f, 0.f), fb0 = fa0;
    float fa4 = 0.f, fb4 = 0.f;
    int row_index = 0;
    if (MODE != PROC_STEP && CK != 2) {
        fa0 = *gather16(a.feat_a, i * (unsigned)(FEAT_STRIDE * 4));
        fb0 = *gather16(a.feat_b, j * (unsigned)(FEAT_STRIDE * 4));
// ... 23 lines not shown
        pair_flow_sums(kc, xi, yj, w, d2, hd.need_d2, acc);
    } else if (MODE == PROC_STEP) {
#ifdef CVO_PROBE_STEP_EXP
        {
            const float d2p = __builtin_fmaf(e2, e2, __builtin_fmaf(e1, e1, e0 * e0));
            const float kp = (float)(kc.s2_d * exp_neg((double)d2p * kc.ninv_2l2, etab ? etab : c_exp2_64));
            asm volatile("" ::"v"(kp));
        }
#endif
        pair_step_sums(kc, xc, yj, e0, e1, e2, w, acc);
    } else {
        if (CK == 2 ? row_index >= 0 : row_index >= first_counted) acc[0] += (double)((kc.inv_l3 * w) * d2);
    }
    return w;
}

template <bool PF>
__device__ __forceinline__ void step_members2(const PairSrc &src, const ProcHead &hd, const KernConsts &kc, const cvo_math::XiConsts &xc,
                                              const CVO_GLOBAL char *kept_w, const float *kept_a, const int packed, const unsigned ebase,
                                              const unsigned wcap, const unsigned n, const int lane, uint2 e, float w, double *acc)
{
    const float *Rt = hd.Rt, *tt = hd.tt;
    uint2 eb = load8(kept_w, min((unsigned)lane + 64u, wcap - 1u));
    for (unsigned off = lane; off < n; off += 128u) {
        const bool two = off + 64u < n;
        if (off >= 128u && !PF) { e = load8(kept_w, off); eb = load8(kept_w, min(off + 64u, wcap - 1u)); }
        float wa = w, wb = 0.0f;
        if (!packed) { wa = kept_a[off]; wb = kept_a[min(off + 64u, wcap - 1u)]; }
        if (!two) { eb = e; wb = wa; }
        unsigned ia, ja, ib, jb;
        float ma, mb;
        kept_unpack(packed, ebase, e, wa, ia, ja, ma);
        kept_unpack(packed, ebase, eb, wb, ib, jb, mb);
        if (!two) mb = 0.0f;
        const float4 xa = load_pos<false>(src.pos_a, ia * 16u), ya = load_pos<false>(src.pos_b, ja * 16u);
        const float4 xb = load_pos<false>(src.pos_a, ib * 16u), yb = load_pos<false>(src.pos_b, jb * 16u);
        if (PF) { e = load8(kept_w, min(off + 128u, wcap - 1u)); eb = load8(kept_w, min(off + 192u, wcap - 1u)); }
        f32x2 px = {xa.x, xb.x}, py = {xa.y, xb.y}, pz = {xa.z, xb.z};
        f32x2 qx = {ya.x, yb.x}, qy = {ya.y, yb.y}, qz = {ya.z, yb.z};
        if (src.tf_a) {
            const f32x2 ox = ((Rt[0] * px + Rt[1] * py) + Rt[2] * pz) + tt[0];
            const f32x2 oy = ((Rt[3] * px + Rt[4] * py) + Rt[5] * pz) + tt[1];
            const f32x2 oz = ((Rt[6] * px + Rt[7] * py) + Rt[8] * pz) + tt[2];
            px = ox; py = oy; pz = oz;
        }
        if (src.tf_b) {
            const f32x2 ox = ((Rt[0] * qx + Rt[1] * qy) + Rt[2] * qz) + tt[0];
            const f32x2 oy = ((Rt[3] * qx + Rt[4] * qy) + Rt[5] * qz) + tt[1];
            const f32x2 oz = ((Rt[6] * qx + Rt[7] * qy) + Rt[8] * qz) + tt[2];
            qx = ox; qy = oy; qz = oz;
        }
        const f32x2 mw = {ma, mb};
        pair_step_sums2(kc, xc, qx, qy, qz, px - qx, py - qy, pz - qz, mw, acc);
    }
}

constexpr int PROC_SMEM = 4 * NACC_MAX * 8 + 4 * PAIR_QUEUE * 8 + 4 * 64 * 8;

template <int MODE, int WEIGHT, int REC, bool PIPE>
__device__ __forceinline__ bool expand_lists(const ProcessArgs &a, const ProcHead &hd, const KernConsts &kc, const unsigned bid, const int wid,
                                             const int lane, const unsigned wave, const int done_word,
                                             const unsigned list_bad, const int in_list, const TileEntry *in_tiles,
                                             const int first_counted, const double *s_etab, uint2 *pairq_all,
                                             double (&acc)[NAcc<MODE>::n])
{
        const bool shared = a.nblk >= NSUB;
        const unsigned nsl = shared ? 1u : (unsigned)(NSUB / a.nblk);
        const unsigned part = shared ? bid / NSUB : 0u;
        unsigned sub = bid & (NSUB - 1);
        unsigned n = list_bad ? 0u : a.st->sub[in_list][sub];
        const TileEntry *tl = in_tiles + (size_t)sub * a.subcap;
        const unsigned stride = shared ? 4u * (unsigned)(a.nblk / NSUB) : 4u;
        const unsigned e0 = part * 4u + (unsigned)wid;
        TileEntry mine = tl[min(e0 + (unsigned)lane * stride, a.subcap - 1)];
        if (done_word != 0) return false;
        uint2 *pairq = pairq_all + wid * PAIR_QUEUE;
        const PairSrc src = pin_pair_src<PIPE>(a);
        int qn = 0;
        unsigned nk = 0;
        unsigned co = 0;
        const size_t kbase = (size_t)wave * a.kept_wcap;
        auto run_batch = [&](int base, int cnt) {
            __builtin_amdgcn_fence(__ATOMIC_RELEASE, "wavefront");
            __builtin_amdgcn_wave_barrier();
            __builtin_amdgcn_fence(__ATOMIC_ACQUIRE, "wavefront");
            float w = 0.0f;
            uint2 pr = make_uint2(0u, 0u);
            float ck = 0.0f;
            float d2 = 0.0f;
            if (lane < cnt) {
                pr = pairq[base + lane];
                w = eval_pair<MODE, WEIGHT, REC>(src, hd, kc, pr.x, pr.y, 0.0f, acc, *hd.xi, s_etab, first_counted, &ck,
                                                 nullptr, nullptr, 0, (REC && MODE == PROC_FLOW) ? &d2 : nullptr);
            }
            if (REC && MODE == PROC_FLOW) {
                const unsigned long long cm = __ballot(lane < cnt && !(d2 >= hd.rec_lim));
                const unsigned add = (unsigned)__popcll(cm);
                if (co + add <= a.kept_wcap) {
                    if (lane < cnt && !(d2 >= hd.rec_lim)) {
                        const unsigned below = __builtin_amdgcn_mbcnt_hi((unsigned)(cm >> 32), __builtin_amdgcn_mbcnt_lo((unsigned)cm, 0u));
                        hd.cand[kbase + co + below] = make_uint2(pr.x | (pr.y << 16), __float_as_uint(ck));
                    }
                } else if (lane == 0) {
                    atomicOr(&a.st->ovf[hd.par][LIST_KEPT], 1u);
                }
                co += add;
// ... 140 lines not shown
        acc[MODE == PROC_FLOW ? 8 : 1] = (double)nk;
        if (NARROW) hd.cand_cnt[wave] = co;
    }
    return true;
}

template <int MODE, int WEIGHT = 0, bool CAND = true, bool PIPE = true>
__device__ __forceinline__ void process_body(const ProcessArgs &a, const unsigned bid, char *scratch, const ProcHead &hd)
{
    if ((int)bid >= a.nblk) return;
    constexpr int NACC = NAcc<MODE>::n;
    double *red = reinterpret_cast<double *>(scratch);
    uint2 *pairq_all = reinterpret_cast<uint2 *>(scratch + 4 * NACC_MAX * 8);
    double *s_etab_all = reinterpret_cast<double *>(scratch + 4 * NACC_MAX * 8 + 4 * PAIR_QUEUE * 8);
#ifdef CVO_PROBE_STEP_EXP
    s_etab_all[threadIdx.x] = c_exp2_64[threadIdx.x & 63];
#else
    if (MODE != PROC_STEP) s_etab_all[threadIdx.x] = c_exp2_64[threadIdx.x & 63];
#endif
    const double *s_etab = s_etab_all + ((MODE == PROC_STEP) ? 0 : (threadIdx.x >> 6) * 64);
    const int tid = threadIdx.x, lane = tid & 63;
    const int wid = __builtin_amdgcn_readfirstlane(tid >> 6);
    const unsigned wave = bid * 4u + (unsigned)wid;
    const int done_word = hd.done_word;
    const KernConsts kc = hd.kc;
    const int first_counted = hd.n_fixed;
    const bool second = hd.second != 0;
    const int in_list = !second ? a.list : (MODE == PROC_FLOW ? (int)LIST_XYB : self_list_id(a.async_self - 1, 1));
    const TileEntry *in_tiles = second ? a.tiles_b : a.tiles;
    const unsigned list_bad = hd.list_bad;

    double acc[NACC];
#pragma unroll
    for (int k = 0; k < NACC; ++k) acc[k] = 0.0;

    if (MODE == PROC_STEP) {
        const size_t base = (size_t)wave * a.kept_wcap;
        unsigned n = a.kept_cnt[wave];
        const int packed = a.kept_packed;
        uint2 e = list_load(&a.kept_ij[base + lane]);
        float w = packed ? 0.0f : a.kept_a[base + lane];
        if (done_word != 0) return;
        if (n > a.kept_wcap) n = a.kept_wcap;
        if (list_bad) n = 0;
        const PairSrc src = pin_pair_src<PIPE>(a);
        const cvo_math::XiConsts xc = xi_uniform(*hd.xi);
        const CVO_GLOBAL char *kept_w = pin_global<PIPE>(a.kept_ij + base);
        const unsigned ebase = pin_u32<PIPE>(a.kept_ebase), wcap = pin_u32<PIPE>(a.kept_wcap);
        constexpr bool PF = PIPE && kPrefetchBuild;
#if defined(CVO_STEP_TWO) && !defined(CVO_PROBE_STEP_EXP)
        step_members2<PF>(src, hd, kc, xc, kept_w, a.kept_a + base, packed, ebase, wcap, n, lane, e, w, acc);
        if (false)
#endif
        for (unsigned off = lane; off < n; off += 64) {
            if (off >= 64) { if (!PF) e = load8(kept_w, off); if (!packed) w = a.kept_a[base + off]; }
            uint2 e_next = e;
            uint2 *const pf = PF ? &e_next : nullptr;
            unsigned mi, mj;
            float mw;
            kept_unpack(packed, ebase, e, w, mi, mj, mw);
#ifdef CVO_PROBE_STEP_EXP
            eval_pair<MODE>(src, hd, kc, mi, mj, mw, acc, xc, s_etab, 0, nullptr, pf, kept_w, min(off + 64u, wcap - 1u));
#else
            eval_pair<MODE>(src, hd, kc, mi, mj, mw, acc, xc, nullptr, 0, nullptr, pf, kept_w, min(off + 64u, wcap - 1u));
#endif
            if (PF) e = e_next;
        }
    } else {
        bool alive;
        if (CAND && WEIGHT == 0 && hd.cand && (MODE == PROC_FLOW ? (!a.async_xy || a.cand_b != nullptr)
                                                                 : (!a.async_self || a.cand_b != nullptr))) {
            if (hd.ck_nblk == a.nblk && MODE == PROC_FLOW && (hd.narrow & REC_NARROW))
                alive = stream_candidates<MODE, PIPE, MODE == PROC_FLOW>(a, hd, kc, lane, wave, done_word, s_etab, acc);
            else if (hd.ck_nblk == a.nblk) alive = stream_candidates<MODE, PIPE>(a, hd, kc, lane, wave, done_word, s_etab, acc);
            else alive = expand_lists<MODE, WEIGHT, WEIGHT == 0 ? 1 : 0, PIPE>(a, hd, kc, bid, wid, lane, wave, done_word, list_bad, in_list, in_tiles, first_counted, s_etab, pairq_all, acc);
        } else {
            alive = expand_lists<MODE, WEIGHT, 0, PIPE>(a, hd, kc, bid, wid, lane, wave, done_word, list_bad, in_list, in_tiles, first_counted, s_etab, pairq_all, acc);
        }
        if (!alive) return;
    }

    wave_sums<NACC>(acc, lane, red + wid * NACC);
    __syncthreads();
    if (tid < NACC) {
        const double s = ((red[tid] + red[NACC + tid]) + red[2 * NACC + tid]) + red[3 * NACC + tid];
        a.partials[(size_t)tid * a.nblk + bid] = s;
    }
}

template <int MODE, int WEIGHT = 0>
__global__ void __launch_bounds__(BLOCK) k_process(const Grp<ProcessArgs> grp)
{
    __shared__ __attribute__((aligned(16))) char scratch[PROC_SMEM];
    const ProcessArgs &a = grp.a[blockIdx.z];
    process_body<MODE, WEIGHT>(a, blockIdx.x, scratch, proc_head_global<MODE>(a, a.st, 0));
}

constexpr int STEP_BLOCK = 1024;
constexpr int STEP_WAVES = STEP_BLOCK / 64;

__device__ __forceinline__ void xi_consts_wave(cvo_math::XiConsts *xi, float *wm, const float omega[3], const float v[3], const int lane)
{
    if (lane == 0) {
        const cvo_math::Mat3 W = cvo_math::skew(omega);
#pragma unroll
        for (int k = 0; k < 9; ++k) wm[k] = W.m[k];
// ... 97 lines not shown
    const bool overflow = s_overflow != 0;
    if (blockIdx.x == 0 && tid == 0) {
        DevState *st = hd;
        if (overflow) {
            st->done = NEED_BIGGER_LIST;
            if (a.done_mirror) *a.done_mirror = NEED_BIGGER_LIST;
        } else {
            for (int q = 0; q < NACC_FLOW; ++q) st->red[RED_FLOW + q] = tot[q];
            for (int q = 0; q < 4; ++q) st->red[RED_XX + q] = a.acvo ? tot[NACC_FLOW + q] : 0.0;
            for (int q = 0; q < 3; ++q) { st->omega[q] = s_xi.omega[q]; st->v[q] = s_xi.v[q]; }
            st->xi = s_xi;
            double dl = 0.0;
            const long long nnz = (long long)tot[8];
            long long nnz_xx = 0, nnz_yy = 0;
            if (a.acvo) {
                nnz_xx = (long long)tot[NACC_FLOW + 1];
                nnz_yy = (long long)tot[NACC_FLOW + 3];
                const double num = (tot[NACC_FLOW + 2] - 2.0 * tot[7]) + tot[NACC_FLOW];
                dl = num / (double)(nnz_xx + nnz_yy - 2 * nnz);
            }
            st->dl = dl;
            if (a.trace && st->k < a.trace_cap) {
                cvo_hip_trace &tr = a.trace[st->k];
                tr.k = st->k;
                tr.exit_code = 0;
                tr.ell = st->ell;
                for (int q = 0; q < 3; ++q) {
                    tr.omega[q] = s_xi.omega[q]; tr.v[q] = s_xi.v[q];
                    tr.omega_d[q] = tot[q]; tr.v_d[q] = tot[3 + q];
                }
                tr.sum_a = tot[6];
                tr.dl = dl;
                tr.nnz = nnz; tr.nnz_xx = nnz_xx; tr.nnz_yy = nnz_yy;
            }
        }
    }
    if (overflow) return false;
    cvo_math::XiConsts xc;
    {
        auto uni = [](float x) { return __int_as_float(__builtin_amdgcn_readfirstlane(__float_as_int(x))); };
#pragma unroll
        for (int q = 0; q < 3; ++q) {
            xc.omega[q] = uni(s_xi.omega[q]); xc.v[q] = uni(s_xi.v[q]);
            xc.u2[q] = uni(s_xi.u2[q]); xc.u3[q] = uni(s_xi.u3[q]); xc.u4[q] = uni(s_xi.u4[q]);
        }
#pragma unroll
        for (int q = 0; q < 9; ++q) {
            xc.W2[q] = uni(s_xi.W2[q]); xc.W3[q] = uni(s_xi.W3[q]); xc.W4[q] = uni(s_xi.W4[q]);
        }
    }

    ProcHead phd;
    phd.need_d2 = 0;
    phd.narrow = 0; phd.rec_lim = PAD_BIG;
    phd.Rt = hd->Rt; phd.tt = hd->t;
    double acc[NACC];
#pragma unroll
    for (int k = 0; k < NACC; ++k) acc[k] = 0.0;
    unsigned wcap = a.kept_wcap, ebase = a.kept_ebase;
    if (n > wcap) n = wcap;
    const PairSrc src = pin_pair_src<true>(a);
    const CVO_GLOBAL char *kept_w = pin_global<true>(a.kept_ij + base);
    wcap = pin_u32<true>(wcap); ebase = pin_u32<true>(ebase);
    constexpr bool PF = kPrefetchBuild;
    for (unsigned off = lane; off < n; off += 64) {
        if (off >= 64) { if (!PF) e = load8(kept_w, off); if (!packed) w = a.kept_a[base + off]; }
        uint2 e_next = e;
        uint2 *const pf = PF ? &e_next : nullptr;
        unsigned mi, mj;
        float mw;
        kept_unpack(packed, ebase, e, w, mi, mj, mw);
        eval_pair<PROC_STEP>(src, phd, kc, mi, mj, mw, acc, xc, nullptr, 0, nullptr, pf, kept_w, min(off + 64u, wcap - 1u));
        if (PF) e = e_next;
    }
    __syncthreads();
    wave_sums<NACC>(acc, lane, sh + wid * NACC);
    __syncthreads();
    if (tid < NACC) {
        double t = 0.0;
#pragma unroll
        for (int q = 0; q < STEP_WAVES; ++q) t += sh[q * NACC + tid];
        a.partials[(size_t)tid * nfat + blockIdx.x] = t;
    }
    return true;
}

__global__ void __launch_bounds__(STEP_BLOCK) k_step_twist(const Grp<ProcessArgs> grp)
{
    step_twist_body(grp.a[blockIdx.z], grp.a[blockIdx.z].st, 0, false);
}

void launch_step_twist_group(const ProcessArgs *a, int n, hipStream_t s, hipEvent_t ev_start, hipEvent_t ev_stop)
{
    Grp<ProcessArgs> g;
    int nblk = 32;
    for (int i = 0; i < n; ++i) { g.a[i] = a[i]; nblk = std::max(nblk, a[i].nblk); }
    const dim3 grid((unsigned)(nblk / (STEP_BLOCK / BLOCK)), 1, (unsigned)n);
    if (ev_start && ev_stop) hipExtLaunchKernelGGL(k_step_twist, grid, dim3(STEP_BLOCK), 0, s, ev_start, ev_stop, 0, g);
    else hipLaunchKernelGGL(k_step_twist, grid, dim3(STEP_BLOCK), 0, s, g);
}

void launch_process_group(int mode, const ProcessArgs *a, int n, hipStream_t s, hipEvent_t ev_start, hipEvent_t ev_stop)
{
    Grp<ProcessArgs> g;
    for (int i = 0; i < n; ++i) g.a[i] = a[i];
    int nblk = 1;
    for (int i = 0; i < n; ++i) nblk = std::max(nblk, a[i].nblk);
// ... 156 lines not shown
            *sh_fail = all_ok ? 0 : 1;
        }
    }
    __syncthreads();
    return *sh_fail == 0;
}

__device__ bool mailbox_allreduce_every_block(const CommTable &ct, DevState *gst, const DevHead *hd, double *vals, int count,
                                              double *sh , int *sh_fail)
{
    __syncthreads();
    const int lane = threadIdx.x;
    if (lane < 64) {
        const unsigned long long seq = hd->mail_snap + 1ull;
        const int gen = (int)(seq & 1ull);
        bool ok = true;
        if (lane < ct.world) {
            if (blockIdx.x == 0) {
                MailSlot *dst = &ct.peer[lane]->slot[gen][ct.rank];
                for (int i = 0; i < count; ++i)
                    __hip_atomic_store(&dst->v[i], vals[i], __ATOMIC_RELAXED, __HIP_MEMORY_SCOPE_SYSTEM);
                __builtin_amdgcn_fence(__ATOMIC_RELEASE, "");
                asm volatile("s_waitcnt vmcnt(0)" ::: "memory");
                __hip_atomic_store(&dst->seq, seq, __ATOMIC_RELAXED, __HIP_MEMORY_SCOPE_SYSTEM);
            }
            const MailSlot *src = &ct.peer[ct.rank]->slot[gen][lane];
            const long long t0 = (long long)wall_clock64();
            while (__hip_atomic_load(&src->seq, __ATOMIC_RELAXED, __HIP_MEMORY_SCOPE_SYSTEM) != seq) {
                if ((long long)wall_clock64() - t0 > ct.timeout_ticks) { ok = false; break; }
                __builtin_amdgcn_s_sleep(8);
            }
            __builtin_amdgcn_fence(__ATOMIC_ACQUIRE, "");
            for (int i = 0; i < count; ++i)
                sh[lane * MAIL_VALS + i] = __hip_atomic_load(&src->v[i], __ATOMIC_RELAXED, __HIP_MEMORY_SCOPE_SYSTEM);
        }
        const bool all_ok = __ballot(!ok) == 0ull;
        __builtin_amdgcn_fence(__ATOMIC_RELEASE, "wavefront");
        __builtin_amdgcn_wave_barrier();
        __builtin_amdgcn_fence(__ATOMIC_ACQUIRE, "wavefront");
        if (lane < count && all_ok) {
            double t = 0.0;
            for (int r = 0; r < ct.world; ++r) t += sh[r * MAIL_VALS + lane];
            vals[lane] = t;
        }
        if (lane == 0) {
            if (blockIdx.x == 0) gst->mail_seq = seq;
            *sh_fail = all_ok ? 0 : 1;
        }
    }
    __syncthreads();
    return *sh_fail == 0;
}

__device__ __forceinline__ void post_flow_body(const PostFlowArgs &a)
{
    __shared__ double sh[4 * NACC_MAX];
    __shared__ __attribute__((aligned(16))) DevHead s_st;
    state_head_to_lds(a.st, &s_st);
    DevHead *st = &s_st;
    if (a.check_done && (st->done != 0 || (a.prm.async_xy && st->stall))) return;
    const bool acvo = a.prm.mode == CVO_HIP_MODE_ACVO;
    if (a.flags & POST_REDUCE) {
        block_reduce_partials<NACC_FLOW>(a.part_flow, a.nblk, sh, st->red + RED_FLOW);
        if (acvo) {
            block_reduce_partials<NACC_SELF>(a.part_xx, a.nblk, sh, st->red + RED_XX);
            block_reduce_partials<NACC_SELF>(a.part_yy, a.nblk, sh, st->red + RED_YY);
        } else if (threadIdx.x == 0) {
            st->red[RED_XX] = st->red[RED_XX + 1] = st->red[RED_YY] = st->red[RED_YY + 1] = 0.0;
        }
        if (threadIdx.x == 0 &&
            ((a.prm.async_xy ? 0u : a.st->ovf[0][LIST_XY]) | a.st->ovf[0][LIST_XX] |
             a.st->ovf[0][LIST_YY] | a.st->ovf[0][LIST_KEPT]))
            st->red[8] = __builtin_nan("");
    }
    bool comm_ok = true;
    if (a.comm) {
        __shared__ double sh_mail[MAX_WORLD * MAIL_VALS];
        __shared__ int sh_fail;
        comm_ok = mailbox_allreduce(*a.comm, a.st, st->red + RED_FLOW, RED_STEP - RED_FLOW, sh_mail, &sh_fail, st);
        if (!comm_ok && threadIdx.x == 0) st->done = DONE_COMM_ERROR;
    }
    if ((a.flags & POST_MATH) && comm_ok && threadIdx.x < 64) {
        const double *red = st->red;
        float omega[3], v[3];
        for (int q = 0; q < 3; ++q) { omega[q] = (float)red[q]; v[q] = (float)red[3 + q]; }
        if (!(red[8] != red[8])) xi_consts_wave(&st->xi, reinterpret_cast<float *>(sh), omega, v, (int)threadIdx.x);
    }
    if ((a.flags & POST_MATH) && comm_ok && threadIdx.x == 0) {
        const bool overflow = st->red[8] != st->red[8];
        if (overflow) st->done = NEED_BIGGER_LIST;
        const double *red = st->red;
        float omega[3], v[3];
        for (int q = 0; q < 3; ++q) {
            omega[q] = (float)red[q];
            v[q] = (float)red[3 + q];
            st->omega[q] = omega[q];
            st->v[q] = v[q];
        }
        double dl = 0.0;
        const long long nnz = (long long)red[8];
        long long nnz_xx = 0, nnz_yy = 0;
        if (acvo) {
            nnz_xx = (long long)red[RED_XX + 1];
            nnz_yy = (long long)red[RED_YY + 1];
            const double num = (red[RED_YY] - 2.0 * red[7]) + red[RED_XX];
            dl = num / (double)(nnz_xx + nnz_yy - 2 * nnz);
        }
        st->dl = dl;
        if (!overflow && a.trace && st->k < a.trace_cap) {
            cvo_hip_trace &tr = a.trace[st->k];
            tr.k = st->k;
            tr.exit_code = 0;
            tr.ell = st->ell;
            for (int q = 0; q < 3; ++q) {
                tr.omega[q] = omega[q]; tr.v[q] = v[q];
                tr.omega_d[q] = red[q]; tr.v_d[q] = red[3 + q];
            }
            tr.sum_a = red[6];
            tr.dl = dl;
            tr.nnz = nnz; tr.nnz_xx = nnz_xx; tr.nnz_yy = nnz_yy;
        }
    }
    __syncthreads();
    if (threadIdx.x == 0 && a.done_mirror && s_st.done != RUNNING) *a.done_mirror = s_st.done;
    state_head_from_lds(&s_st, a.st);
}

__global__ void __launch_bounds__(BLOCK) k_post_flow(const Grp<PostFlowArgs> grp)
{
    post_flow_body(grp.a[blockIdx.z]);
}

enum HeadMode { HM_CLASSIC = 0, HM_HEAD = 1 };

template <int HM>
__device__ __forceinline__ void head_post(DevHead *lds, const PostStepArgs &a, const bool run_post, const bool publisher, const bool timed,
                                          long long (&clk)[4], const cvo_math::ExpPre *pre = nullptr )
{
    const DevParams &p = a.prm;
    const bool acvo = p.mode == CVO_HIP_MODE_ACVO;
    const bool lane0 = (threadIdx.x & 63) == 0;
    const bool was_pending = HM == HM_CLASSIC ? true : (lds->pending != 0);
    float R[9], T[3], Rt[9], t[3], omega[3], v[3];
#pragma unroll
    for (int q = 0; q < 9; ++q) { R[q] = lds->R[q]; Rt[q] = lds->Rt[q]; }
#pragma unroll
    for (int q = 0; q < 3; ++q) { T[q] = lds->T[q]; t[q] = lds->t[q]; omega[q] = lds->omega[q]; v[q] = lds->v[q]; }
    float ell = lds->ell, ell_max = lds->ell_max;
    const double dl = lds->dl;
    double bcde[4];
#pragma unroll
    for (int q = 0; q < 4; ++q) bcde[q] = lds->red[RED_STEP + q];
    int k = lds->k, done = lds->done, iter = lds->iter, n_exec = lds->n_exec;
    const int n_slots = lds->n_slots + (was_pending ? 1 : 0);
    if (run_post) {
        if (timed) clk[0] = (long long)__builtin_readcyclecounter();
        const cvo_math::CubicBracket cb = cvo_math::cubic_bracket(bcde);
        const float step = cvo_math::finish_step(
            cb.found, cb.found ? section_root_wave(cb, (int)(threadIdx.x & 63)) : 0.0, p.min_step);
        if (timed) clk[1] = (long long)__builtin_readcyclecounter();
        cvo_hip_trace *tr = (publisher && lane0 && a.trace && k < a.trace_cap) ? &a.trace[k] : nullptr;
// ... 310 lines not shown
{
    if (init.on) {
        static_assert(DEVSTATE_INIT_BYTES % 4 == 0, "word stores");
        uint32_t *z = reinterpret_cast<uint32_t *>(st);
        for (int q = threadIdx.x; q < (int)(DEVSTATE_INIT_BYTES / 4); q += BLOCK) z[q] = 0u;
        __syncthreads();
        if (threadIdx.x == 0) {
            for (int q = 0; q < 9; ++q) st->R[q] = init.R[q];
            for (int q = 0; q < 3; ++q) { st->T[q] = init.T[q]; st->center[q] = init.center[q]; }
            st->ell = init.ell; st->ell_max = init.ell_max;
            st->iter = init.iter; st->n_fixed = init.n_fixed; st->done = init.done;
            st->xmax = init.xmax; st->y0max = init.y0max;
        }
        __syncthreads();
    }
    if (build_masks && threadIdx.x < 4) build_masks[threadIdx.x] = 0xffffffffu;
    for (int q = threadIdx.x; q < LIST_N * NSUB; q += BLOCK) (&st->sub[0][0])[q] = 0u;
    if (threadIdx.x < 16) (&st->ovf[0][0])[threadIdx.x] = 0u;
    if (threadIdx.x == 0) {
        for (int l = 0; l < 3; ++l) {
            st->list_ok[l] = 0;
            atomicOr(&st->built[l][(st->k >> 5) & 63], 1u << (st->k & 31));
        }
        for (int l = 0; l < 2; ++l) {
            st->sf_ok[l][0] = st->sf_ok[l][1] = 0;
            st->sf_ck[l][0] = st->sf_ck[l][1] = 0;
            st->sf_active[l] = 0; st->sf_target[l] = -1; st->sf_fresh[l] = -1;
        }
        st->xy_ok[0] = st->xy_ok[1] = 0;
        st->xy_ck[0] = st->xy_ck[1] = 0;
        st->rec_count[0] = st->rec_count[1] = 0;
        st->xy_active = 0;
        st->xy_target = -1;
        st->xy_fresh = -1;
        st->stall = 0;
        st->pending = 0;
        st->mail_snap = st->mail_seq;
        prepare_iteration(st, st, true, prm, plan_builds_none());
        count_async_plan(st, st, prm);
    }
}

void launch_prepare(DevState *st, const DevParams &prm, hipStream_t s, uint32_t *build_masks, const PrepareInit *init)
{
    PrepareInit in{};
    if (init) in = *init;
    hipLaunchKernelGGL(k_prepare, dim3(1), dim3(BLOCK), 0, s, st, prm, build_masks, in);
}

void launch_post_flow_group(const PostFlowArgs *a, int n, hipStream_t s)
{
    Grp<PostFlowArgs> g;
    for (int i = 0; i < n; ++i) g.a[i] = a[i];
    hipLaunchKernelGGL(k_post_flow, dim3(1, 1, (unsigned)n), dim3(BLOCK), 0, s, g);
}

void launch_post_step_group(const PostStepArgs *a, int n, hipStream_t s)
{
    Grp<PostStepArgs> g;
    for (int i = 0; i < n; ++i) g.a[i] = a[i];
    hipLaunchKernelGGL(k_post_step, dim3(1, 1, (unsigned)n), dim3(BLOCK), 0, s, g);
}

typedef const __attribute__((address_space(4))) Slot *CSlot;
#define CVO_SLOT(tab)                          \
    CSlot cs = (CSlot)(tab) + blockIdx.z;      \
    if (cs->active == 0) return
#define CVO_ARG(T, field) (*(const T *)(&cs->field))
#define CVO_FILTER_ROLE(role) (*(const FilterArgs *)(&cs->op[q + (role)].f))

__global__ void __launch_bounds__(BLOCK) __attribute__((amdgpu_waves_per_eu(6, 8)))
kt_filter(const Slot *__restrict__ tab, const int ql)
{
    const int q = ql & QP_MASK, list = (ql >> 8) & 3;
    typedef const __attribute__((address_space(4))) uint32_t *CMask;
    const CMask masks = (CMask)(reinterpret_cast<const char *>(tab) - kTableHeaderBytes);
    const bool may_build = ((masks[list] >> blockIdx.z) & 1u) != 0u;
    constexpr unsigned PT_BLOCKS = 64;
    if (!may_build && blockIdx.x >= PT_BLOCKS) return;
    CVO_SLOT(tab);
    if (may_build) filter_body(CVO_ARG(FilterArgs, op[q].f), blockIdx.x, gridDim.x, cs->op[q].f.st, 0);
    if (blockIdx.x < PT_BLOCKS)
        pretransform_body(CVO_ARG(FilterArgs, op[q].f), blockIdx.x, min(gridDim.x, PT_BLOCKS));
}

__global__ void __launch_bounds__(BLOCK) __attribute__((amdgpu_waves_per_eu(6, 8)))
kt_filter_group(const Slot *__restrict__ tab, const int q)
{
    typedef const __attribute__((address_space(4))) uint32_t *CMask;
    const CMask masks = (CMask)(reinterpret_cast<const char *>(tab) - kTableHeaderBytes);
    const bool may_build = ((masks[blockIdx.y] >> blockIdx.z) & 1u) != 0u;
    constexpr unsigned PT_BLOCKS = 64;
    if (!may_build && (blockIdx.y != 0 || blockIdx.x >= PT_BLOCKS)) return;
    CVO_SLOT(tab);
    if (may_build) filter_body(CVO_FILTER_ROLE((int)blockIdx.y), blockIdx.x, gridDim.x, cs->op[q + (int)blockIdx.y].f.st, 0);
    if (blockIdx.y == 0 && blockIdx.x < PT_BLOCKS) pretransform_body(CVO_FILTER_ROLE(0), blockIdx.x, min(gridDim.x, PT_BLOCKS));
}

#ifndef CVO_FLOW_WAVES
#define CVO_FLOW_WAVES 5
#endif
template <int MODE, int WEIGHT = 0>
__global__ void __launch_bounds__(BLOCK) __attribute__((amdgpu_waves_per_eu((MODE == PROC_FLOW && WEIGHT == 0) ? CVO_FLOW_WAVES : 1, 8)))
kt_process(const Slot *__restrict__ tab, const int q)
{
    __shared__ __attribute__((aligned(16))) char scratch[PROC_SMEM];
    CVO_SLOT(tab);
// ... 95 lines not shown
        CVO_SLOT(tab);                                                                                     \
        int b = (int)blockIdx.x;                                                                           \
        const int np = cs->op[q].np;                                                                       \
        if (b < np) {                                                                                      \
            const ProcessArgs &pa = CVO_ARG(ProcessArgs, op[q].p);                                         \
            process_body<PROC_FLOW, 0, false, false>(pa, (unsigned)b, smem, proc_head_global<PROC_FLOW>(pa, pa.st, 0)); \
            return;                                                                                        \
        }                                                                                                  \
        b -= np;                                                                                           \
        if (b < 2 * np) {                                                                                  \
            const int w = b >= np ? 1 : 0;                                                                 \
            const ProcessArgs &pa = CVO_ARG(ProcessArgs, op[q + 1 + w].p);                                 \
               \
            process_body<PROC_SELF, 0, false, false>(pa, (unsigned)(b - w * np), smem, proc_head_global<PROC_SELF>(pa, pa.st, 0)); \
            return;                                                                                        \
        }                                                                                                  \
        b -= 2 * np;                                                                                       \
        const int n0 = cs->op[q].n0, n1 = cs->op[q].n1;                                                    \
        const int role = b < n0 ? 0 : (b < n0 + n1 ? 1 : 2);                                               \
        filter_body<false>(CVO_FILTER_ROLE(role), (unsigned)(b - (role == 0 ? 0 : (role == 1 ? n0 : n0 + n1))),   \
                    (unsigned)(role == 0 ? n0 : (role == 1 ? n1 : cs->op[q].n2)), cs->op[q + role].f.st, 0); \
    }
CVO_MERGED_KERNELS(_w4, 4)

template <int MODE>
__device__ __forceinline__ ProcHead proc_head_lds(const ProcessArgs &a, const DevHead *h, const int par, float (&rt)[12])
{
    auto uni = [](float x) { return __int_as_float(__builtin_amdgcn_readfirstlane(__float_as_int(x))); };
    auto unid = [](double x) {
        return __hiloint2double(__builtin_amdgcn_readfirstlane(__double2hiint(x)), __builtin_amdgcn_readfirstlane(__double2loint(x)));
    };
    ProcHead hd;
#pragma unroll
    for (int q = 0; q < 9; ++q) rt[q] = uni(h->Rt[q]);
#pragma unroll
    for (int q = 0; q < 3; ++q) rt[9 + q] = uni(h->t[q]);
    hd.Rt = rt; hd.tt = rt + 9; hd.xi = nullptr;
    const KernConsts &k = h->kc;
    hd.kc.tau = uni(k.tau); hd.kc.tau_c = uni(k.tau_c); hd.kc.sp = uni(k.sp);
    hd.kc.inv_c = uni(k.inv_c); hd.kc.inv_d = uni(k.inv_d); hd.kc.inv_l3 = uni(k.inv_l3);
    hd.kc.cb = uni(k.cb); hd.kc.cg = uni(k.cg); hd.kc.cd = uni(k.cd); hd.kc.cscale = uni(k.cscale);
    hd.kc.s2_d = unid(k.s2_d); hd.kc.cs2_d = unid(k.cs2_d);
    hd.kc.ninv_2l2 = unid(k.ninv_2l2); hd.kc.ninv_2cl2 = unid(k.ninv_2cl2);
    hd.done_word = 0;
    hd.n_fixed = (MODE == PROC_SELF && a.first_counted) ? __builtin_amdgcn_readfirstlane(h->n_fixed) : 0;
    hd.second = ((MODE == PROC_FLOW && __builtin_amdgcn_readfirstlane(h->xy_active) == 1) ||
                 (MODE == PROC_SELF && __builtin_amdgcn_readfirstlane(h->sf_active[a.async_self == 2 ? 1 : 0]) == 1)) ? 1 : 0;
    hd.list_bad = 0u;
    hd.ck_nblk = 0;
    hd.par = par;
    hd.cand = nullptr; hd.cand_cnt = nullptr;
    hd.need_d2 = a.need_d2;
    hd.narrow = 0; hd.rec_lim = PAD_BIG;
    if (a.cand_b) {
        const int l = a.async_self == 2 ? 1 : 0;
        const int ck = MODE == PROC_FLOW ? (hd.second ? h->xy_ck[1] : h->xy_ck[0]) : (hd.second ? h->sf_ck[l][1] : h->sf_ck[l][0]);
        hd.ck_nblk = __builtin_amdgcn_readfirstlane(ck);
        hd.cand = hd.second ? a.cand_b : a.cand;
        hd.cand_cnt = hd.second ? a.cand_cnt_b : a.cand_cnt;
    }
    return hd;
}

#define CVO_SLOT_HEAD(tab)                                                                                    \
    CSlot cs = (CSlot)(tab) + blockIdx.z;                                                                     \
    const int q = qp & QP_MASK, par = (qp & QP_PARITY) ? 1 : 0;                                               \
    {                                                                                                         \
        const PostStepArgs &hps = CVO_ARG(PostStepArgs, op[q].ps);                                            \
        const int active = cs->active, np_ = cs->op[q].np, hn = hps.nblk, hcd = hps.check_done;               \
        const DevState *hst = hps.st, *hst2 = hps.st2;                                                        \
        const double *hpart = hps.part_step;                                                                  \
        const long long *hdbg = hps.dbg;                                                                      \
        asm volatile("" ::"s"(active), "s"(np_), "s"(hn), "s"(hcd), "s"(hst), "s"(hst2), "s"(hpart), "s"(hdbg)); \
        if (active == 0) return;                                                                              \
    }
#define CVO_HEAD_KERNELS(SUFFIX, WAVES)                                                                    \
    __global__ void __launch_bounds__(BLOCK) __attribute__((amdgpu_waves_per_eu(WAVES, 8)))               \
    kt_hflow_build##SUFFIX(const Slot *__restrict__ tab, const int qp)                                     \
    {                                                                                                      \
        extern __shared__ __attribute__((aligned(16))) char smem[];                                        \
        __shared__ double sh[4 * NACC_MAX];                                                                \
        __shared__ __attribute__((aligned(16))) DevHead s_st;                                              \
        CVO_SLOT_HEAD(tab);                                                                                \
        const int np = cs->op[q].np;                                                                       \
        if ((int)blockIdx.x >= np) {                                                                       \
            const FilterArgs &f = CVO_ARG(FilterArgs, op[q].f);                                            \
            filter_body<false>(f, blockIdx.x - (unsigned)np, (unsigned)cs->op[q].n0, par ? f.st2 : f.st, par);    \
            return;                                                                                        \
        }                                                                                                  \
        const PostStepArgs ps = CVO_ARG(PostStepArgs, op[q].ps);                                           \
        const ProcessArgs &pa = CVO_ARG(ProcessArgs, op[q].p);                                             \
        if (!head_body<HM_HEAD>(ps, par ? ps.st2 : ps.st, par ? ps.st : ps.st2, &s_st, sh, par,            \
                                blockIdx.x == 0, &pa)) return;                                             \
        float rt[12];                                                                                      \
        process_body<PROC_FLOW, 0, true, false>(pa, blockIdx.x, smem, proc_head_lds<PROC_FLOW>(pa, &s_st, par, rt)); \
        if (ps.dbg && blockIdx.x == 0 && threadIdx.x == 0 && ps.dbg[6] != 0) {    \
            ps.dbg[7] += (long long)__builtin_readcyclecounter() - ps.dbg[6];                              \
            ps.dbg[6] = 0;                                                                                 \
        }                                                                                                  \
    }                                                                                                      \
    __global__ void __launch_bounds__(BLOCK) __attribute__((amdgpu_waves_per_eu(WAVES, 8)))               \
    kt_hflow_build6##SUFFIX(const Slot *__restrict__ tab, const int qp)                                    \
    {                                                                                                      \
        extern __shared__ __attribute__((aligned(16))) char smem[];                                        \
        __shared__ double sh[4 * NACC_MAX];                                                                \
        __shared__ __attribute__((aligned(16))) DevHead s_st;                                              \
// ... 1169 lines not shown
__global__ void __launch_bounds__(RUN_BLOCK) __attribute__((amdgpu_waves_per_eu(2, 2)))
kt_run(const Slot *__restrict__ tab, const int qs)
{
    extern __shared__ __attribute__((aligned(16))) float4 s_lc[];
    run_body<false>(tab, qs, s_lc);
}
__global__ void __launch_bounds__(RUN_BLOCK) __attribute__((amdgpu_waves_per_eu(2, 2)))
kt_run_acvo(const Slot *__restrict__ tab, const int qs)
{
    run_body<true>(tab, qs, nullptr);
}
__global__ void __launch_bounds__(RUN_BLOCK) __attribute__((amdgpu_waves_per_eu(2, 2)))
kt_run_side(const Slot *__restrict__ tab, const int qs)
{
    extern __shared__ __attribute__((aligned(16))) float4 s_lc[];
    run_body<false, true>(tab, qs, s_lc);
}
__global__ void __launch_bounds__(RUN_BLOCK) __attribute__((amdgpu_waves_per_eu(2, 2)))
kt_run_acvo_side(const Slot *__restrict__ tab, const int qs)
{
    run_body<true, true>(tab, qs, nullptr);
}

__global__ void __launch_bounds__(BLOCK) __attribute__((amdgpu_waves_per_eu(4, 8)))
kt_side_filter(const Slot *__restrict__ tab, const int q)
{
    CSlot cs = (CSlot)(tab);
    if (cs->active == 0) return;
    const FilterArgs &f = CVO_ARG(FilterArgs, op[q].f);
    filter_body<false>(f, blockIdx.x, gridDim.x, f.st2, 1);
}
__global__ void __launch_bounds__(BLOCK) __attribute__((amdgpu_waves_per_eu(4, 8)))
kt_side_record(const Slot *__restrict__ tab, const int q)
{
    __shared__ __attribute__((aligned(16))) char scratch[PROC_SMEM];
    CSlot cs = (CSlot)(tab);
    if (cs->active == 0) return;
    const ProcessArgs &pa = CVO_ARG(ProcessArgs, op[q].p);
    RunMail *const mail = CVO_ARG(PostStepArgs, op[q].ps).run_mail;
    const DevState *h = pa.st2;
    const int t = __builtin_amdgcn_readfirstlane(h->xy_target);
    if (t >= 0 && mail != nullptr) {
        ProcHead hd;
        hd.Rt = h->Rt; hd.tt = h->t; hd.xi = &h->xi;
        hd.kc = h->kc;
        hd.done_word = 0; hd.n_fixed = 0;
        hd.second = t ? 1 : 0;
        hd.list_bad = 0u;
        hd.ck_nblk = 0;
        hd.par = 1;
        hd.cand = t ? pa.cand_b : pa.cand;
        hd.cand_cnt = t ? pa.cand_cnt_b : pa.cand_cnt;
        hd.need_d2 = 0;
        hd.narrow = 0; hd.rec_lim = PAD_BIG;
        process_body<PROC_FLOW, 0, true, false>(pa, blockIdx.x, scratch, hd);
    }
    __threadfence();
    __syncthreads();
    if (threadIdx.x == 0 && mail != nullptr)
        __hip_atomic_fetch_add(&mail->side_done, 1ull, __ATOMIC_RELEASE, __HIP_MEMORY_SCOPE_AGENT);
}

unsigned filter_grid_cap(long long nitems, long long cap) { return filter_grid_x(nitems, cap); }
long long filter_blocks_cap() { return filter_blocks_max(); }

void launch_table(const Slot *tab, const TLaunch &l, hipStream_t s, hipEvent_t ev_start, hipEvent_t ev_stop, int parity)
{
    const dim3 g(l.gx, 1, l.gz);
    const int qp = l.q | (parity ? QP_PARITY : 0) | QP_HEAD;
    if (ev_start && ev_stop && (l.kernel == TK_FLOW || l.kernel == TK_FLOW_D2)) {
        if (l.kernel == TK_FLOW_D2) hipExtLaunchKernelGGL(kt_flow_d2, g, dim3(BLOCK), 0, s, ev_start, ev_stop, 0, tab, l.q);
        else hipExtLaunchKernelGGL(kt_process<PROC_FLOW>, g, dim3(BLOCK), 0, s, ev_start, ev_stop, 0, tab, l.q);
        return;
    }
    switch (l.kernel) {
    case TK_FILTER: hipLaunchKernelGGL(kt_filter, g, dim3(BLOCK), l.smem, s, tab, l.q | (l.list << 8)); break;
    case TK_FILTER_GROUP: hipLaunchKernelGGL(kt_filter_group, dim3(l.gx, 3, l.gz), dim3(BLOCK), l.smem, s, tab, l.q); break;
    case TK_FLOW: hipLaunchKernelGGL(kt_process<PROC_FLOW>, g, dim3(BLOCK), 0, s, tab, l.q); break;
    case TK_FLOW_D2: hipLaunchKernelGGL(kt_flow_d2, g, dim3(BLOCK), 0, s, tab, l.q); break;
    case TK_FLOW_MATLAB: hipLaunchKernelGGL((kt_process<PROC_FLOW, 1>), g, dim3(BLOCK), 0, s, tab, l.q); break;
    case TK_STEP: hipLaunchKernelGGL(kt_process<PROC_STEP>, g, dim3(BLOCK), 0, s, tab, l.q); break;
    case TK_SELF: hipLaunchKernelGGL(kt_process<PROC_SELF>, g, dim3(BLOCK), 0, s, tab, l.q); break;
    case TK_SELF2: hipLaunchKernelGGL(kt_self2, dim3(l.gx, 2, l.gz), dim3(BLOCK), 0, s, tab, l.q); break;
    case TK_STEP_TWIST: hipLaunchKernelGGL(kt_step_twist, g, dim3(STEP_BLOCK), 0, s, tab, l.q); break;
    case TK_FLOW_BUILD: hipLaunchKernelGGL(kt_flow_build_w4, g, dim3(BLOCK), l.smem, s, tab, l.q); break;
    case TK_FLOW_BUILD3: hipLaunchKernelGGL(kt_flow_build3_w4, g, dim3(BLOCK), l.smem, s, tab, l.q); break;
    case TK_FLOW_BUILD6: hipLaunchKernelGGL(kt_flow_build6_w4, g, dim3(BLOCK), l.smem, s, tab, l.q); break;
    case TK_POST_FLOW: hipLaunchKernelGGL(kt_post_flow, g, dim3(BLOCK), 0, s, tab, l.q); break;
    case TK_POST_STEP: hipLaunchKernelGGL(kt_post_step, g, dim3(BLOCK), 0, s, tab, l.q); break;
    case TK_HFLOW_BUILD: hipLaunchKernelGGL(kt_hflow_build_w4, g, dim3(BLOCK), l.smem, s, tab, qp); break;
    case TK_HFLOW_BUILD6: hipLaunchKernelGGL(kt_hflow_build6_w4, g, dim3(BLOCK), l.smem, s, tab, qp); break;
    case TK_HSTEP_TWIST: hipLaunchKernelGGL(kt_step_twist, g, dim3(STEP_BLOCK), 0, s, tab, qp); break;
    case TK_RUN:
        if (l.list) hipLaunchKernelGGL(kt_run_side, dim3(l.gx), dim3(RUN_BLOCK), RUN_LDS_BYTES, s, tab, l.q);
        else hipLaunchKernelGGL(kt_run, dim3(l.gx), dim3(RUN_BLOCK), RUN_LDS_BYTES, s, tab, l.q);
        break;
    case TK_RUN_ACVO:
        if (l.list) hipLaunchKernelGGL(kt_run_acvo_side, dim3(l.gx), dim3(RUN_BLOCK), 0, s, tab, l.q);
        else hipLaunchKernelGGL(kt_run_acvo, dim3(l.gx), dim3(RUN_BLOCK), 0, s, tab, l.q);
        break;
    case TK_SIDE_FILTER: hipLaunchKernelGGL(kt_side_filter, g, dim3(BLOCK), l.smem, s, tab, l.q); break;
    case TK_SIDE_RECORD: hipLaunchKernelGGL(kt_side_record, g, dim3(BLOCK), 0, s, tab, l.q); break;
    default: break;
    }
}

void launch_post_flow(const PostFlowArgs &a, hipStream_t s) { launch_post_flow_group(&a, 1, s); }
// ... 4 lines not shown
```

### cvo-rgbd_amd/csrc/cvo_plan.cpp

```cpp
#include "cvo_internal.h"

using namespace cvo_dev;
using namespace cvo_impl;

namespace cvo_impl {

FilterPlan plan_filter(int nrows, int nb)
{
    FilterPlan p{};
    const int tiles = std::max(1, (nrows + ROWS_PER_TILE - 1) / ROWS_PER_TILE);
    const int want_blocks = 4096;
    const int chunks_want = std::max(1, (want_blocks + tiles / 2) / tiles);
    int jt = (nb + chunks_want - 1) / chunks_want;
    jt = std::max(jt, 64);
    jt = std::min(jt, 2048);
    jt = (jt + SEG - 1) & ~(SEG - 1);
    p.jt = jt;
    const int chunks = std::max(1, (nb + jt - 1) / jt);
    p.grid = dim3(chunks, tiles);
    return p;
}

int ensure_buf(cvo_hip_ctx *ctx, DevBuf &b, size_t bytes)
{
// ... 185 lines not shown
    KeptView v{};
    v.kept_ij = (const uint2 *)ctx->lists[LIST_KEPT].a.p;
    v.kept_a = (const float *)ctx->lists[LIST_KEPT].b.p;
    v.kept_cnt = (const uint32_t *)ctx->kept_cnt.p;
    v.st = ctx->st;
    v.nblk = ctx->proc_blocks;
    v.kept_wcap = ctx->lists[LIST_KEPT].cap / (uint32_t)(4 * ctx->proc_blocks);
    v.kept_packed = kept_format(ctx, &v.kept_ebase);
    return v;
}

int enqueue_process(cvo_hip_ctx *ctx, int mode, int list, DevBuf &part, const float4 *pos_a,
                    const float *feat_a, int tf_a, const float4 *pos_b, const float *feat_b,
                    int tf_b, int first_counted, int check_done)
{
    int rc = ensure_buf(ctx, part, (size_t)PROC_WAVES * NACC_MAX * sizeof(double));
    if (rc) return rc;
    rc = ensure_list(ctx, list, 0, 0, 0);
    if (rc) return rc;
    if (!ctx->kept_cnt.p) {
        rc = ensure_buf(ctx, ctx->kept_cnt, PROC_WAVES * sizeof(uint32_t));
        if (rc) return rc;
        HIP_TRY(ctx, hipMemsetAsync(ctx->kept_cnt.p, 0, PROC_WAVES * sizeof(uint32_t), ctx->stream));
    }
    if (mode == PROC_FLOW)
        rc = ensure_list(ctx, LIST_KEPT, ctx->fixed.np, ctx->moving.np, 0);
    else
        rc = ensure_list(ctx, LIST_KEPT, 0, 0, 0);
    if (rc) return rc;
    ProcessArgs a{};
    a.pos_a = pos_a; a.feat_a = feat_a;
    a.pos_b = pos_b; a.feat_b = feat_b;
    a.tiles = (const TileEntry *)ctx->lists[list].a.p;
    a.kept_ij = (uint2 *)ctx->lists[LIST_KEPT].a.p;
    a.kept_a = (float *)ctx->lists[LIST_KEPT].b.p;
    a.kept_cnt = (uint32_t *)ctx->kept_cnt.p;
    a.partials = (double *)part.p;
    a.st = ctx->st;
    a.st2 = static_cast<DevState *>(ctx->st2);
    a.subcap = ctx->lists[list].cap / NSUB;
    a.nblk = ctx->proc_blocks;
    a.kept_wcap = ctx->lists[LIST_KEPT].cap / (uint32_t)(4 * ctx->proc_blocks);
    a.list = list;
    a.first_counted = first_counted;
    a.tf_a = tf_a; a.tf_b = tf_b;
    if (pre_transform(ctx) && ctx->pos_bt.p) {
        if (tf_b && pos_b == ctx->moving.pos) { a.pos_b = (const float4 *)ctx->pos_bt.p; a.tf_b = 0; }
        if (tf_a && pos_a == ctx->moving.pos) { a.pos_a = (const float4 *)ctx->pos_bt.p; a.tf_a = 0; }
    }
    a.check_done = check_done;
    a.need_d2 = (ctx->prm.mode == CVO_HIP_MODE_ACVO || !ctx->in_loop || ctx->cur_trace_cap > 0) ? 1 : 0;
    a.weight = ctx->prm.color_scale > 0.0f ? 1 : 0;
    a.kept_packed = kept_format(ctx, &a.kept_ebase);
    if ((mode == PROC_FLOW && list == LIST_XY) || (mode == PROC_SELF && (list == LIST_XX || list == LIST_YY))) {
        const bool no_cand = ctx->opt.no_cand;
        ctx->ck_nblk[list] = 0;
        if (!no_cand && pre_transform(ctx) && !(ctx->prm.color_scale > 0.0f) && a.kept_packed == 1) {
            int rc_c = ensure_buf(ctx, ctx->cand[list], (size_t)ctx->lists[LIST_KEPT].cap * sizeof(uint2));
            if (!rc_c) rc_c = ensure_buf(ctx, ctx->cand_cnt[list], PROC_WAVES * sizeof(uint32_t));
            if (!rc_c) {
                a.cand = (uint2 *)ctx->cand[list].p;
                a.cand_cnt = (uint32_t *)ctx->cand_cnt[list].p;
                ctx->ck_nblk[list] = a.nblk;
            } else {
                (void)hipGetLastError();
                ctx->err = "";
            }
        }
    }
    if (ctx->in_loop && ctx->use_async) {
        a.async_xy = 1;
        a.tiles_b = (const TileEntry *)ctx->lists[LIST_XYB].a.p;
        const bool no_cand = ctx->opt.no_cand;
        if (mode == PROC_FLOW && list == LIST_XY && ctx->plan_recording && ctx->lone && ctx->allow_head && !multi_rank(ctx) &&
            !no_cand && a.kept_packed == 1 && !(ctx->prm.color_scale > 0.0f)) {
            const size_t bytes = (size_t)ctx->lists[LIST_KEPT].cap * sizeof(uint2);
            int rc_c = ensure_buf(ctx, ctx->cand[LIST_XY], bytes);
            if (!rc_c) rc_c = ensure_buf(ctx, ctx->cand_xyb, bytes);
            if (!rc_c) rc_c = ensure_buf(ctx, ctx->cand_cnt[LIST_XY], PROC_WAVES * sizeof(uint32_t));
            if (!rc_c) rc_c = ensure_buf(ctx, ctx->cand_cnt_xyb, PROC_WAVES * sizeof(uint32_t));
            if (!rc_c) {
                a.cand = (uint2 *)ctx->cand[LIST_XY].p;
                a.cand_cnt = (uint32_t *)ctx->cand_cnt[LIST_XY].p;
                a.cand_b = (uint2 *)ctx->cand_xyb.p;
                a.cand_cnt_b = (uint32_t *)ctx->cand_cnt_xyb.p;
                ctx->ck_nblk[LIST_XY] = a.nblk;
            } else {
                (void)hipGetLastError();
                ctx->err = "";
            }
        }
    }
    if (mode == PROC_SELF && ctx->in_loop && ctx->use_async_self) {
        a.async_self = list == LIST_XX ? 1 : 2;
        a.tiles_b = (const TileEntry *)ctx->lists[list == LIST_XX ? LIST_XXB : LIST_YYB].a.p;
        const bool no_cand = ctx->opt.no_cand;
        if (ctx->plan_recording && ctx->lone && ctx->allow_head && !multi_rank(ctx) && !no_cand && a.kept_packed == 1 &&
            !(ctx->prm.color_scale > 0.0f)) {
            const int l = list == LIST_XX ? 0 : 1;
            const size_t bytes = (size_t)ctx->lists[LIST_KEPT].cap * sizeof(uint2);
            int rc_c = ensure_buf(ctx, ctx->cand[list], bytes);
            if (!rc_c) rc_c = ensure_buf(ctx, ctx->cand_sfb[l], bytes);
            if (!rc_c) rc_c = ensure_buf(ctx, ctx->cand_cnt[list], PROC_WAVES * sizeof(uint32_t));
            if (!rc_c) rc_c = ensure_buf(ctx, ctx->cand_cnt_sfb[l], PROC_WAVES * sizeof(uint32_t));
            if (!rc_c) {
                a.cand = (uint2 *)ctx->cand[list].p;
                a.cand_cnt = (uint32_t *)ctx->cand_cnt[list].p;
                a.cand_b = (uint2 *)ctx->cand_sfb[l].p;
                a.cand_cnt_b = (uint32_t *)ctx->cand_cnt_sfb[l].p;
                ctx->ck_nblk[list] = a.nblk;
            } else {
                (void)hipGetLastError();
                ctx->err = "";
            }
        }
    }
    const bool twist = mode == PROC_STEP && ctx->merge_twist;
    if (twist) {
        a.flow_part = (const double *)ctx->part_flow.p;
        a.xx_part = (const double *)ctx->part_xx.p;
        a.yy_part = (const double *)ctx->part_yy.p;
        a.trace = ctx->cur_trace; a.trace_cap = ctx->cur_trace_cap;
        a.acvo = ctx->prm.mode == CVO_HIP_MODE_ACVO;
        a.done_mirror = ctx->done_mirror;
        a.comm = ctx->comm_table;
    }
    const bool build = mode == PROC_FLOW && ctx->have_xy_build;
    ctx->have_xy_build = ctx->have_xy_build && mode != PROC_FLOW;
    if (ctx->rec) {
        RecOp op; op.kind = RecOp::PROCESS; op.mode = twist ? kProcStepTwist : (build ? kFlowBuild : mode);
        op.p = a;
        if (build) op.f = ctx->xy_build;
        ctx->rec->push_back(op);
        return CVO_HIP_OK;
    }
    EventPair ev{};
    const bool timed = ctx->profiling && !build && (mode == PROC_FLOW || mode == PROC_STEP);
    if (timed) {
        HIP_TRY(ctx, hipEventCreate(&ev.a));
        HIP_TRY(ctx, hipEventCreate(&ev.b));
        ev.kind = mode == PROC_FLOW ? kEvProcFlow : kEvProcStep;
        ev.iter_tag = ctx->iter_tag;
        ev.pairs = 0.0;
    }
    if (build) return fail(ctx, CVO_HIP_ERR_INVALID, "asynchronous build outside the table path");
    if (twist) launch_step_twist_group(&a, 1, ctx->stream, ev.a, ev.b);
    else launch_process(mode, a, ctx->stream, ev.a, ev.b);
    if (timed) ctx->events.push_back(ev);
    HIP_TRY(ctx, hipGetLastError());
    return CVO_HIP_OK;
}

void emit_post_flow(cvo_hip_ctx *ctx, const PostFlowArgs &pa)
{
    if (ctx->rec) {
        RecOp op; op.kind = RecOp::POST_FLOW; op.pf = pa;
        ctx->rec->push_back(op);
    } else {
        launch_post_flow(pa, ctx->stream);
    }
}

void emit_post_step(cvo_hip_ctx *ctx, const PostStepArgs &pa)
{
    if (ctx->rec) {
        RecOp op; op.kind = RecOp::POST_STEP; op.ps = pa;
        ctx->rec->push_back(op);
    } else {
        launch_post_step(pa, ctx->stream);
    }
}

int drain_events(cvo_hip_ctx *ctx, int n_exec, const DevState *fin)
{
    for (auto &ev : ctx->events) {
        float ms = 0.f;
        HIP_TRY(ctx, hipEventSynchronize(ev.b));
        HIP_TRY(ctx, hipEventElapsedTime(&ms, ev.a, ev.b));
        bool live = !(n_exec >= 0 && ev.iter_tag >= n_exec);
        if (live && fin && ev.iter_tag >= 0 && ev.kind >= 0 && ev.kind < 3)
            live = (fin->built[ev.kind][(ev.iter_tag >> 5) & 63] >> (ev.iter_tag & 31)) & 1u;
        if (!live) {
        } else if (ev.kind == kEvProcFlow) {
            ctx->prof.proc_flow_ms += ms; ctx->prof.proc_flow_launches++;
        } else if (ev.kind == kEvProcStep) {
            ctx->prof.step_ms += ms; ctx->prof.step_launches++;
        } else if (ev.kind == LIST_XY) {
            ctx->prof.flow_ms += ms; ctx->prof.flow_launches++; ctx->prof.flow_pairs += ev.pairs;
        } else {
            ctx->prof.self_ms += ms; ctx->prof.self_launches++; ctx->prof.self_pairs += ev.pairs;
        }
        (void)hipEventDestroy(ev.a);
        (void)hipEventDestroy(ev.b);
    }
    ctx->events.clear();
    return CVO_HIP_OK;
}

bool host_reduce(const cvo_hip_ctx *ctx) { return !ctx->comm_table && (ctx->comm || ctx->user_allreduce); }
bool multi_rank(const cvo_hip_ctx *ctx) { return ctx->comm_table || ctx->comm || ctx->user_allreduce; }

DevParams loop_params(const cvo_hip_ctx *ctx)
{
    DevParams dp = ctx->dprm;
    dp.list_margin = ((double)ctx->fixed.n * (double)ctx->moving.n <= 2.0e8) ? 0.25f : 0.15f;
// ... 50 lines not shown
            rc = enqueue_filter(ctx, LIST_YY, ctx->moving, slo, shi, tfm, ctx->moving, tfm, check_done);
        if (!rc)
            rc = enqueue_process(ctx, PROC_SELF, LIST_YY, ctx->part_yy, ctx->moving.pos,
                                 ctx->moving.feat, tfm, ctx->moving.pos, ctx->moving.feat, tfm,
                                 1 , check_done);
    }
    if (group_lists) {
        ctx->rec = nullptr;
        if (!rc) {
            FilterArgs f[3], build{}, ahead[2];
            ProcessArgs flow{}, self[2];
            int nf = 0, ns = 0, na = 0;
            bool have_flow = false, have_build = false;
            for (const RecOp &op : local) {
                if (op.kind == RecOp::FILTER && op.mode == kFilterAhead && na < 2) ahead[na++] = op.f;
                else if (op.kind == RecOp::FILTER && nf < 3) f[nf++] = op.f;
                else if (op.kind == RecOp::PROCESS && (op.mode == PROC_FLOW || op.mode == kFlowBuild)) {
                    flow = op.p; have_flow = true;
                    if (op.mode == kFlowBuild) { build = op.f; have_build = true; }
                }
                else if (op.kind == RecOp::PROCESS && op.mode == PROC_SELF && ns < 2) self[ns++] = op.p;
            }
            if (nf) launch_filter_group(f, nf, ctx->stream);
            if (have_flow && !have_build) launch_process_group(PROC_FLOW, &flow, 1, ctx->stream);
            else if (have_flow) rc = fail(ctx, CVO_HIP_ERR_INVALID, "asynchronous build outside the table path");
            if (ns) launch_process_group(PROC_SELF, self, ns, ctx->stream);
            HIP_TRY(ctx, hipGetLastError());
        }
    }
    if (rc) return rc;
    if (ctx->merge_twist) return CVO_HIP_OK;
    PostFlowArgs pa{};
    pa.st = ctx->st;
    pa.prm = ctx->in_loop ? loop_params(ctx) : ctx->dprm;
    pa.trace = trace; pa.trace_cap = trace_cap;
    pa.check_done = check_done;
    pa.done_mirror = ctx->done_mirror;
    pa.nblk = ctx->proc_blocks;
    pa.part_flow = (const double *)ctx->part_flow.p;
    pa.part_xx = (const double *)ctx->part_xx.p;
    pa.part_yy = (const double *)ctx->part_yy.p;
    pa.comm = ctx->comm_table;
    if (host_reduce(ctx)) {
        pa.flags = POST_REDUCE;
        emit_post_flow(ctx, pa);
        rc = reduce_over_ranks(ctx, RED_FLOW, RED_STEP - RED_FLOW);
        if (rc) return rc;
        if (do_math) {
            pa.flags = POST_MATH;
            emit_post_flow(ctx, pa);
        }
    } else {
        pa.flags = POST_REDUCE | (do_math ? POST_MATH : 0);
        emit_post_flow(ctx, pa);
    }
    HIP_TRY(ctx, hipGetLastError());
    return CVO_HIP_OK;
}

int enqueue_step(cvo_hip_ctx *ctx, int check_done, bool do_math, cvo_hip_trace *trace,
                 int trace_cap)
{
    int rc = enqueue_process(ctx, PROC_STEP, LIST_XY, ctx->part_step, ctx->fixed.pos,
                             ctx->fixed.feat, 0, ctx->moving.pos, ctx->moving.feat, 1, 0,
                             check_done);
    if (rc) return rc;
    PostStepArgs pa{};
    pa.st = ctx->st;
    pa.st2 = static_cast<DevState *>(ctx->st2);
    pa.prm = ctx->in_loop ? loop_params(ctx) : ctx->dprm;
    pa.trace = trace; pa.trace_cap = trace_cap;
    pa.check_done = check_done;
    pa.done_mirror = ctx->done_mirror;
    pa.progress_mirror = ctx->progress_mirror;
    for (int l = 0; l < 3; ++l) pa.ck_nblk[l] = ctx->plan_recording ? ctx->ck_nblk[l] : 0;
    pa.nblk = ctx->merge_twist ? ctx->proc_blocks / STEP_TWIST_ROWS_DIV : ctx->proc_blocks;
    pa.part_step = (const double *)ctx->part_step.p;
    pa.dbg = ctx->post_dbg;
    pa.comm = ctx->comm_table;
    if (ctx->plan_recording && ctx->lone && ctx->allow_head && runs_allowed(ctx) && ctx->use_async && ctx->merge_twist &&
        !multi_rank(ctx) && (ctx->prm.mode == CVO_HIP_MODE_CVO || (ctx->use_async_self && !ctx->opt.no_acvo_run)) &&
        !(ctx->prm.color_scale > 0.0f) && !ctx->post_dbg) {
        const bool fresh = ctx->run_mail.p == nullptr;
        if (ensure_buf(ctx, ctx->run_mail, sizeof(RunMail)) == CVO_HIP_OK) {
            if (fresh) HIP_TRY(ctx, hipMemsetAsync(ctx->run_mail.p, 0, sizeof(RunMail), loop_stream(ctx)));
            pa.run_mail = (RunMail *)ctx->run_mail.p;
            pa.run_mirror = ctx->run_mirror;
            pa.run_iters = 64;
            pa.run_g_max = std::max(8, std::min(ctx->run_g_max, ctx->run_g_call));
            pa.run_timeout_ticks = (long long)(ctx->opt.run_timeout_ms * 1.0e5);
            pa.run_fault = ctx->opt.run_fault;
            if (!ctx->opt.no_side_builds) {
                if (!ctx->side_stream && hipStreamCreateWithFlags(&ctx->side_stream, hipStreamNonBlocking) != hipSuccess) {
                    (void)hipGetLastError();
                    ctx->side_stream = nullptr;
                }
                if (ctx->side_stream) {
                    pa.side_mirror = ctx->side_mirror;
                    pa.run_build_at = ctx->opt.run_build_at;
                }
            }
        } else {
            (void)hipGetLastError();
            ctx->err = "";
        }
    }
// ... 170 lines not shown
                slot.op[q + i].f = f[i];
                gx = std::max(gx, filter_grid_cap(filter_items(f[i]), cap));
                jt = std::max(jt, f[i].jt);
            }
            plan.push_back(mk_launch(TK_FILTER_GROUP, q, gx, 1, smem_of(jt)));
            q += 3;
        } else {
            for (int i = 0; i < nf; ++i) {
                slot.op[q].f = f[i];
                plan.push_back(mk_launch(TK_FILTER, q, filter_grid_cap(filter_items(f[i]), fbmax), 1, smem_of(f[i].jt)));
                plan.back().list = f[i].list;
                ++q;
            }
        }
        if (have_flow && have_build) {
            OpArgs &o = slot.op[q];
            o.p = flow; o.f = build;
            const long long cap = std::max<long long>(64, fbmax / 2);
            o.np = std::max(8, flow.nblk);
            o.n0 = (int)std::max(8u, filter_grid_cap(filter_items(build), cap));
            if (head) { o.ps = ops[at + 1].ps; }
            else { o.ps.run_mail = nullptr; }
            plan.push_back(mk_launch(head ? TK_HFLOW_BUILD : TK_FLOW_BUILD, q, (unsigned)(o.np + o.n0), 1,
                                     head ? smem_head(build.jt) : smem_of(build.jt)));
            if (head && pre && o.ps.run_mail && flow.cand && flow.cand_b && flow.kept_packed == 1 && flow.tf_a == 0 && flow.tf_b == 1 &&
                flow.weight == 0 && 4 * flow.nblk <= PROC_WAVES) {
                pre->push_back(mk_launch(TK_RUN, q | ((q + 1) << 4), 1u + (unsigned)std::max(8, std::min((int)RUN_G, o.ps.run_g_max)), 1));
                pre->push_back(mk_launch(TK_RUN, q | ((q + 1) << 4), 1u + RUN_G_SMALL, 1));
                if (side && o.ps.side_mirror && o.f.st2) {
                    side->push_back(mk_launch(TK_SIDE_FILTER, q, (unsigned)o.n0, 1, smem_of(build.jt)));
                    side->push_back(mk_launch(TK_SIDE_RECORD, q, (unsigned)o.np, 1));
                }
            }
            ++q;
        } else if (have_flow) {
            slot.op[q].p = flow;
            plan.push_back(mk_launch(flow.weight == 1 ? TK_FLOW_MATLAB : (flow.need_d2 ? TK_FLOW_D2 : TK_FLOW), q, (unsigned)std::max(1, flow.nblk), 1));
            ++q;
        }
    }
    if (ns == 2) {
        slot.op[q].p = self[0]; slot.op[q + 1].p = self[1];
        plan.push_back(mk_launch(TK_SELF2, q, (unsigned)std::max(self[0].nblk, self[1].nblk), 1));
        q += 2;
    } else if (ns == 1) {
        slot.op[q].p = self[0];
        plan.push_back(mk_launch(TK_SELF, q, (unsigned)self[0].nblk, 1));
        ++q;
    }
    for (; at < ops.size(); ++at) {
        if (q >= MAX_OPS) return false;
        const RecOp &op = ops[at];
        OpArgs &o = slot.op[q];
        if (op.kind == RecOp::POST_FLOW) { o.pf = op.pf; plan.push_back(mk_launch(TK_POST_FLOW, q, 1, 1)); }
        else if (op.kind == RecOp::POST_STEP) {
            o.ps = op.ps;
            if (have_flow && flow.async_xy) o.ps.ck_nblk[LIST_XY] = 0;
            for (int w = 0; w < 2; ++w)
                if (ns_all > w && self_async[w]) o.ps.ck_nblk[LIST_XX + w] = 0;
            plan.push_back(mk_launch(TK_POST_STEP, q, 1, 1));
        }
        else if (op.kind == RecOp::PROCESS && op.mode == kProcStepTwist) {
            o.p = op.p;
            plan.push_back(mk_launch(head ? TK_HSTEP_TWIST : TK_STEP_TWIST, q, (unsigned)std::max(8, std::max(32, op.p.nblk) / 4), 1));
            if (head) { ++q; break; }
        } else if (op.kind == RecOp::PROCESS && op.mode == PROC_STEP) {
            o.p = op.p;
            plan.push_back(mk_launch(TK_STEP, q, (unsigned)std::max(1, op.p.nblk), 1));
        } else return false;
        ++q;
    }
    *head_mode = head;
    return q <= MAX_OPS;
}

bool plan_fused(const std::vector<const std::vector<RecOp> *> &ops, const std::vector<Slot *> &slots, int zdim,
                std::vector<TLaunch> &plan)
{
    plan.clear();
    if (ops.empty()) return true;
    const size_t nq = ops[0]->size();
    if (nq > (size_t)MAX_OPS) return false;
    for (const auto *o : ops)
        if (o->size() != nq) return false;
    const long long fbmax = filter_blocks_cap();
    std::vector<size_t> perm(nq);
    for (size_t q = 0; q < nq; ++q) perm[q] = q;
    {
        const std::vector<RecOp> &r = *ops[0];
        auto is_f = [&](size_t q) { return q < nq && r[q].kind == RecOp::FILTER && r[q].mode != kFilterAhead; };
        auto is_p = [&](size_t q, int mode) { return q < nq && r[q].kind == RecOp::PROCESS && r[q].mode == mode; };
        if (is_f(0) && is_p(1, PROC_FLOW) && is_f(2) && is_p(3, PROC_SELF) && is_f(4) && is_p(5, PROC_SELF)) {
            const size_t order[6] = {0, 2, 4, 1, 3, 5};
            for (size_t q = 0; q < 6; ++q) perm[q] = order[q];
        }
    }
    for (size_t qs = 0; qs < nq; ++qs) {
        const size_t q = perm[qs];
        const RecOp &first = (*ops[0])[q];
        for (const auto *o : ops)
            if ((*o)[q].kind != first.kind || (*o)[q].mode != first.mode) return false;
        unsigned gx = 1, smem = 0;
        int kernel = -1, np = 8;
        unsigned nfb = 8;
        for (size_t i = 0; i < ops.size(); ++i) {
            const RecOp &op = (*ops[i])[q];
            OpArgs &o = slots[i]->op[qs];
            switch (op.kind) {
            case RecOp::FILTER: {
                o.f = op.f;
                kernel = TK_FILTER;
                const long long cap = std::max<long long>(kFusedFilterBlocks, fbmax / (2 * zdim));
                gx = std::max(gx, filter_grid_cap(filter_items(op.f), cap));
                smem = std::max(smem, (unsigned)filter_smem_bytes(op.f.jt));
                break;
            }
            case RecOp::PROCESS:
                o.p = op.p;
                if (op.mode == kProcStepTwist) {
                    kernel = TK_STEP_TWIST;
                    gx = std::max(gx, (unsigned)(std::max(32, op.p.nblk) / 4));
                } else if (op.mode == kFlowBuild) {
                    kernel = TK_FLOW_BUILD;
                    o.f = op.f;
                    const long long cap = std::max<long long>(64, fbmax / (2 * zdim));
                    np = std::max(np, op.p.nblk);
                    nfb = std::max(nfb, filter_grid_cap(filter_items(op.f), cap));
                    smem = std::max(smem, (unsigned)filter_smem_bytes(op.f.jt));
                } else {
                    kernel = op.mode == PROC_FLOW ? (op.p.weight == 1 ? TK_FLOW_MATLAB : TK_FLOW)
                                                  : (op.mode == PROC_STEP ? TK_STEP : TK_SELF);
                    gx = std::max(gx, (unsigned)op.p.nblk);
                }
                break;
            case RecOp::POST_FLOW: o.pf = op.pf; kernel = TK_POST_FLOW; break;
            case RecOp::POST_STEP: o.ps = op.ps; kernel = TK_POST_STEP; break;
            }
        }
        if (kernel == TK_FLOW) {
            bool d2 = false;
            for (size_t i = 0; i < ops.size(); ++i) d2 = d2 || (*ops[i])[q].p.need_d2 != 0;
            if (d2) kernel = TK_FLOW_D2;
        }
        if (kernel == TK_FLOW_BUILD) {
            gx = (unsigned)np + nfb;
            for (Slot *sl : slots) { sl->op[qs].np = np; sl->op[qs].n0 = (int)nfb; }
        }
        plan.push_back(mk_launch(kernel, (int)qs, gx, (unsigned)zdim, smem));
        if (kernel == TK_FILTER) plan.back().list = first.f.list;
    }
    std::vector<TLaunch> merged;
    for (size_t i = 0; i < plan.size(); ++i) {
        auto run_of = [&](int kernel, size_t n) {
            if (i + n > plan.size()) return false;
            for (size_t k = 0; k < n; ++k)
                if (plan[i + k].kernel != kernel || plan[i + k].q != plan[i].q + (int)k) return false;
            return true;
        };
        if (run_of(TK_FILTER, 3)) {
            TLaunch l = plan[i];
            l.kernel = TK_FILTER_GROUP;
            for (size_t k = 1; k < 3; ++k) { l.gx = std::max(l.gx, plan[i + k].gx); l.smem = std::max(l.smem, plan[i + k].smem); }
            merged.push_back(l);
            i += 2;
        } else if (run_of(TK_SELF, 2)) {
            TLaunch l = plan[i];
            l.kernel = TK_SELF2;
            l.gx = std::max(l.gx, plan[i + 1].gx);
            merged.push_back(l);
            i += 1;
        } else {
            merged.push_back(plan[i]);
        }
    }
    plan.swap(merged);
    return true;
}

void set_build_masks(Slot &slot, const std::vector<TLaunch> &plan, uint32_t *masks, int z)
{
    bool filters = false;
    for (const TLaunch &l : plan) filters = filters || l.kernel == TK_FILTER || l.kernel == TK_FILTER_GROUP;
    for (const TLaunch &l : plan)
        if (l.kernel == TK_POST_STEP) {
            slot.op[l.q].ps.build_mask = filters ? masks : nullptr;
            slot.op[l.q].ps.slot_bit = 1u << z;
        }
}
// ... 187 lines not shown
```

Baseline: 4300 registrations/s.

## Precompute per-moving-point step terms into a table reused across kept pairs

Adds a per-moving-point table of xi-dependent step coefficients, filled by extra blocks of the post-flow kernel once the twist is known. The step kernel then loads four float4 rows per pair instead of recomputing the W2/W3/W4 matrix products for every kept pair. The table is only used when the average number of kept members per moving point reaches a configurable threshold. The cost is extra memory traffic, an extra table buffer, wider post-flow launches and a duplicated partial reduction in those extra blocks.

```diff
diff --git a/cvo-rgbd_amd/csrc/cvo_capi.cpp b/cvo-rgbd_amd/csrc/cvo_capi.cpp
--- a/cvo-rgbd_amd/csrc/cvo_capi.cpp
+++ b/cvo-rgbd_amd/csrc/cvo_capi.cpp
@@ -42,6 +42,7 @@
     {"engine_crowd", "CVO_HIP_ENGINE_CROWD", 2, 0.0},     {"engine_merge_max", "CVO_HIP_ENGINE_MERGE_MAX", 2, 0.0},
     {"matches_combine", nullptr, 0, 0.0},                 {"scan_chunk", nullptr, 0, 0.0},
     {"record_narrow", "CVO_HIP_NO_RECORD_NARROW", 1, 0.0}, {"list_stale_max", "CVO_HIP_LIST_STALE_MAX", 2, 0.0},
+    {"step_table_min", "CVO_HIP_STEP_TABLE_MIN", 2, 0.0},
 };
 void env_defaults(cvo_hip_ctx *ctx)
 {
@@ -96,6 +97,7 @@
     else if (is("list_margin")) { if (v > 4.0) return CVO_HIP_ERR_INVALID; o.list_margin = v < 0.0 ? -1.0f : (float)v; }
     else if (is("record_narrow")) o.record_narrow = on;
     else if (is("list_stale_max")) { if (!(v >= 1.0 && v <= 64.0)) return CVO_HIP_ERR_INVALID; o.list_stale_max = (float)v; }
+    else if (is("step_table_min")) { if (!(v == v) || v > 1.0e6) return CVO_HIP_ERR_INVALID; o.step_table_min = v < 0.0 ? -1.0f : (float)v; }
     else if (is("final_mirror")) o.no_final_mirror = !on;
     else if (is("twist_on_shared_gpu")) o.twist_on_shared_gpu = on;
     else if (is("comm_debug")) o.comm_debug = on;
@@ -348,7 +350,7 @@
                     (void *)ctx->moving.feat, (void *)ctx->fixed.seg, (void *)ctx->moving.seg,
                     (void *)ctx->scratch_a.pos, (void *)ctx->scratch_a.feat, (void *)ctx->scratch_a.seg,
                     (void *)ctx->scratch_b.pos, (void *)ctx->scratch_b.feat, (void *)ctx->scratch_b.seg, (void *)ctx->st, (void *)ctx->st2, ctx->part_flow.p, ctx->part_xx.p,
-                    ctx->part_yy.p, ctx->part_step.p, ctx->part_hess.p, ctx->part_score.p, ctx->part_matches.p, ctx->run_mail.p, (void *)ctx->trace_dev, ctx->kept_cnt.p, ctx->pos_bt.p, ctx->cand[0].p, ctx->cand[1].p, ctx->cand[2].p, ctx->cand_xyb.p, ctx->cand_cnt_xyb.p, ctx->cand_sfb[0].p, ctx->cand_sfb[1].p, ctx->cand_cnt_sfb[0].p, ctx->cand_cnt_sfb[1].p, ctx->cand_cnt[0].p,
+                    ctx->part_yy.p, ctx->part_step.p, ctx->part_hess.p, ctx->part_score.p, ctx->part_matches.p, ctx->run_mail.p, (void *)ctx->trace_dev, ctx->kept_cnt.p, ctx->pos_bt.p, ctx->step_tab.p, ctx->cand[0].p, ctx->cand[1].p, ctx->cand[2].p, ctx->cand_xyb.p, ctx->cand_cnt_xyb.p, ctx->cand_sfb[0].p, ctx->cand_sfb[1].p, ctx->cand_cnt_sfb[0].p, ctx->cand_cnt_sfb[1].p, ctx->cand_cnt[0].p,
                     ctx->cand_cnt[1].p, ctx->cand_cnt[2].p})
         if (p) (void)hipFree(p);
     for (int l = 0; l < LIST_N; ++l) {
@@ -624,7 +626,8 @@
         if (!rc) rc = check_overflow_and_grow(ctx, &redo);
         if (rc) return rc;
     }
-    rc = enqueue_step(ctx, 0, false, nullptr, 0);
+    rc = enqueue_step_table(ctx);
+    if (!rc) rc = enqueue_step(ctx, 0, false, nullptr, 0);
     if (rc) return rc;
     rc = fetch_red(ctx, RED_STEP, 4, bcde);
     if (!rc && ctx->profiling) rc = drain_events(ctx);
@@ -851,6 +854,7 @@
     else if (is("list_margin")) *value = o.list_margin;
     else if (is("record_narrow")) *value = o.record_narrow;
     else if (is("list_stale_max")) *value = o.list_stale_max;
+    else if (is("step_table_min")) *value = o.step_table_min;
     else if (is("final_mirror")) *value = !o.no_final_mirror;
     else if (is("twist_on_shared_gpu")) *value = o.twist_on_shared_gpu;
     else if (is("comm_debug")) *value = o.comm_debug;
@@ -867,6 +871,7 @@
     else if (is("list_grows")) *value = (double)ctx->list_grows;
     else if (is("async_builds_named")) *value = (double)ctx->async_stats[0];
     else if (is("async_stalls")) *value = (double)ctx->async_stats[1];
+    else if (is("step_table_passes")) *value = (double)ctx->step_table_passes;
     else if (is("run_aborts")) *value = (double)ctx->run_aborts;
     else if (is("no_run_backoff")) *value = ctx->no_run_backoff;
     else return CVO_HIP_ERR_INVALID;
diff --git a/cvo-rgbd_amd/csrc/cvo_device.h b/cvo-rgbd_amd/csrc/cvo_device.h
--- a/cvo-rgbd_amd/csrc/cvo_device.h
+++ b/cvo-rgbd_amd/csrc/cvo_device.h
@@ -138,7 +138,7 @@
     float xmax, y0max;
     float tauf[3];
     int32_t n_fixed;
-    uint32_t pad0_;
+    int32_t step_tab_passes;
     float list_r[3];
     int32_t list_ok[3];
     int32_t reuse[3];
@@ -149,7 +149,7 @@
     float rec_Rt[9], rec_t[3];
     int32_t list_stat[3];
     int32_t async_stat[2];
-    int32_t rec_pad_;
+    int32_t step_tab_on;
     int32_t xy_active, xy_target, stall, xy_fresh;
     int32_t xy_ok[2];
     int32_t xy_ck[2];
@@ -264,6 +264,8 @@
     const CommTable *comm;
     int kept_packed;
     unsigned kept_ebase;
+    const float4 *step_tab;
+    unsigned step_tab_rows;
 };
 
 enum { POST_REDUCE = 1, POST_MATH = 2 };
@@ -279,8 +281,15 @@
     int32_t *done_mirror;
     int nblk;
     const CommTable *comm;
+    float4 *step_tab;
+    const float4 *tab_pos;
+    unsigned tab_rows;
+    int tab_tf;
+    float tab_min;
+    int tab_xi;
     DevParams prm;
 };
+constexpr int STEP_TAB_BLOCKS = 8;
 
 struct PostStepArgs {
     DevState *st;
diff --git a/cvo-rgbd_amd/csrc/cvo_internal.h b/cvo-rgbd_amd/csrc/cvo_internal.h
--- a/cvo-rgbd_amd/csrc/cvo_internal.h
+++ b/cvo-rgbd_amd/csrc/cvo_internal.h
@@ -195,6 +195,8 @@
 using namespace cvo_dev;
 using namespace cvo_impl;
 
+constexpr float kStepTableMinDefault = 2.0f;
+
 struct CtxOptions {
     bool no_cand = false;
     bool no_graph = false;
@@ -224,6 +226,7 @@
     double list_init = 0.0;
     float list_margin = -1.0f;
     bool record_narrow = true;
+    float step_table_min = kStepTableMinDefault;
     float list_stale_max = 3.0f;
     int run_cand = 0;
     double mailbox_timeout_s = 5.0;
@@ -239,6 +242,7 @@
     long long tail_handovers = 0;
     long long run_aborts = 0;
     int list_stats[3] = {0, 0, 0};
+    int step_table_passes = 0;
     int async_stats[2] = {0, 0};
     long long list_grows = 0;
     long long run_timeouts = 0;
@@ -290,6 +294,8 @@
     DevBuf cand_xyb, cand_cnt_xyb;
     DevBuf cand_sfb[2], cand_cnt_sfb[2];
     int ck_nblk[3] = {0, 0, 0};
+    DevBuf step_tab;
+    bool step_tab_armed = false;
     DevBuf pos_bt;
     bool lone = true;
     bool allow_async_self = true;
@@ -408,6 +414,7 @@
 int prepare_buffers(cvo_hip_ctx *ctx);
 int enqueue_iterations(cvo_hip_ctx *ctx, int count, int tag0, int trace_cap);
 void drop_graphs(cvo_hip_ctx *ctx);
+int enqueue_step_table(cvo_hip_ctx *ctx);
 TLaunch mk_launch(int kernel, int q, unsigned gx, unsigned gz, unsigned smem = 0);
 bool plan_lone(const std::vector<RecOp> &ops, Slot &slot, std::vector<TLaunch> &plan, const bool allow_head, bool *head_mode,
                std::vector<TLaunch> *pre = nullptr, std::vector<TLaunch> *side = nullptr);
diff --git a/cvo-rgbd_amd/csrc/cvo_job.cpp b/cvo-rgbd_amd/csrc/cvo_job.cpp
--- a/cvo-rgbd_amd/csrc/cvo_job.cpp
+++ b/cvo-rgbd_amd/csrc/cvo_job.cpp
@@ -186,6 +186,7 @@
     const int executed = f.n_exec;
     for (int q = 0; q < 3; ++q) ctx->list_stats[q] = f.list_stat[q];
     for (int q = 0; q < 2; ++q) ctx->async_stats[q] = f.async_stat[q];
+    ctx->step_table_passes = f.step_tab_passes;
     if (j.trace_cap > 0 && executed > 0)
         HIP_TRY(ctx, hipMemcpy(j.trace, ctx->trace_dev,
                                (size_t)std::min(executed, j.trace_cap) * sizeof(cvo_hip_trace),
diff --git a/cvo-rgbd_amd/csrc/cvo_kernels.hip b/cvo-rgbd_amd/csrc/cvo_kernels.hip
--- a/cvo-rgbd_amd/csrc/cvo_kernels.hip
+++ b/cvo-rgbd_amd/csrc/cvo_kernels.hip
@@ -4,15 +4,12 @@
 
 #include "cvo_device.h"
 #include "cvo_pair.h"
+#include "cvo_step.h"
 
 namespace cvo_dev {
 
 typedef float f32x4 __attribute__((ext_vector_type(4)));
 
-__device__ __forceinline__ float mv_row(const float *m, float x, float y, float z)
-{
-    return (m[0] * x + m[1] * y) + m[2] * z;
-}
 
 constexpr int FILTER_KMAX = 64;
 size_t filter_smem_bytes(int jt)
@@ -345,14 +342,6 @@
 template <> struct NAcc<PROC_STEP> { static constexpr int n = NACC_STEP; };
 template <> struct NAcc<PROC_SELF> { static constexpr int n = NACC_SELF; };
 
-__device__ __forceinline__ double div6(double x)
-{
-    const double c = 0x1.5555555555555p-3;
-    const double q0 = x * c;
-    const double r = __builtin_fma(-6.0, q0, x);
-    return __builtin_fma(r, c, q0);
-}
-
 __device__ __forceinline__ uint2 list_load(const uint2 *p)
 {
 #ifdef CVO_NT_LISTS
@@ -384,6 +373,7 @@
     int need_d2;
     int narrow;
     float rec_lim;
+    int step_tab;
 };
 
 template <int MODE>
@@ -404,6 +394,7 @@
     h.need_d2 = a.need_d2;
     h.narrow = (MODE == PROC_FLOW && !a.async_xy) ? st->narrow : 0;
     h.rec_lim = (h.narrow & REC_BOUNDED) ? st->rec_r * st->rec_r : PAD_BIG;
+    h.step_tab = (MODE == PROC_STEP && a.step_tab) ? st->step_tab_on : 0;
     return h;
 }
 
@@ -494,53 +485,13 @@
 #endif
 }
 
-__device__ __forceinline__ void step_tail(const float w, const float beta, const float gamma, const float delta, const float epsil, double *acc)
-{
-    const double A = (double)w;
-    const double b = (double)beta, g = (double)gamma;
-    acc[0] += (double)(w * beta);
-#ifdef CVO_STEP_TAIL_LITERAL
-    acc[1] += A * (g + (double)(beta * beta) / 2.0);
-    acc[2] += A * ((double)(delta + beta * gamma) + div6((double)(beta * beta * beta)));
-    acc[3] += A * ((((double)(epsil + beta * delta) + 0.5 * b * b * g) + 0.5 * g * g) +
-                   1 / 24.0 * b * b * b * b);
-#else
-    acc[1] = __builtin_fma(A, __builtin_fma((double)(beta * beta), 0.5, g), acc[1]);
-    acc[2] = __builtin_fma(A, __builtin_fma((double)(beta * beta * beta), 0x1.5555555555555p-3,
-                                            (double)(delta + beta * gamma)), acc[2]);
-    const double b2 = b * b, hg = 0.5 * g;
-    double t = __builtin_fma(b2, hg, (double)(epsil + beta * delta));
-    t = __builtin_fma(hg, g, t);
-    t = __builtin_fma(b2 * (1 / 24.0), b2, t);
-    acc[3] = __builtin_fma(A, t, acc[3]);
-#endif
-}
-
-__device__ __forceinline__ void pair_step_sums(const KernConsts &kc, const cvo_math::XiConsts &xc, const float4 yj, const float e0,
+template <class XI>
+__device__ __forceinline__ void pair_step_sums(const KernConsts &kc, const XI &xc, const float4 yj, const float e0,
                                            const float e1, const float e2, const float w, double *acc)
 {
-    float xiz[3], xi2z[3], xi3z[3], xi4z[3];
-    xiz[0] = (xc.omega[1] * yj.z - xc.omega[2] * yj.y) + xc.v[0];
-    xiz[1] = (xc.omega[2] * yj.x - xc.omega[0] * yj.z) + xc.v[1];
-    xiz[2] = (xc.omega[0] * yj.y - xc.omega[1] * yj.x) + xc.v[2];
-#pragma unroll
-    for (int r = 0; r < 3; ++r) {
-        xi2z[r] = mv_row(xc.W2 + 3 * r, yj.x, yj.y, yj.z) + xc.u2[r];
-        xi3z[r] = mv_row(xc.W3 + 3 * r, yj.x, yj.y, yj.z) + xc.u3[r];
-        xi4z[r] = mv_row(xc.W4 + 3 * r, yj.x, yj.y, yj.z) + xc.u4[r];
-    }
-    const float normxiz2 = (xiz[0] * xiz[0] + xiz[1] * xiz[1]) + xiz[2] * xiz[2];
-    const float xz12 = -((xiz[0] * xi2z[0] + xiz[1] * xi2z[1]) + xiz[2] * xi2z[2]);
-    const float eps_c = ((xi2z[0] * xi2z[0] + xi2z[1] * xi2z[1]) + xi2z[2] * xi2z[2]) +
-                        2 * ((xiz[0] * xi3z[0] + xiz[1] * xi3z[1]) + xiz[2] * xi3z[2]);
-    const float cb = kc.cb, cg = kc.cg, cd = kc.cd;
-    const float beta = ((cb * xiz[0]) * e0 + (cb * xiz[1]) * e1) + (cb * xiz[2]) * e2;
-    const float g_dot = ((2.0f * xi2z[0]) * e0 + (2.0f * xi2z[1]) * e1) + (2.0f * xi2z[2]) * e2;
-    const float gamma = cg * (normxiz2 + g_dot);
-    const float d_dot = ((-xi3z[0]) * e0 + (-xi3z[1]) * e1) + (-xi3z[2]) * e2;
-    const float delta = cd * (xz12 + d_dot);
-    const float e_dot = ((2.0f * xi4z[0]) * e0 + (2.0f * xi4z[1]) * e1) + (2.0f * xi4z[2]) * e2;
-    const float epsil = cg * (eps_c + e_dot);
+    const StepPoint P = step_point_terms(kc, xc, yj.x, yj.y, yj.z);
+    float beta, gamma, delta, epsil;
+    step_member_terms(kc, P, e0, e1, e2, beta, gamma, delta, epsil);
     step_tail(w, beta, gamma, delta, epsil, acc);
 }
 
@@ -670,6 +621,39 @@
         }
         const f32x2 mw = {ma, mb};
         pair_step_sums2(kc, xc, qx, qy, qz, px - qx, py - qy, pz - qz, mw, acc);
+    }
+}
+
+template <bool PF>
+__device__ __forceinline__ void step_members_table(const PairSrc &src, const ProcHead &hd, const KernConsts &kc, const CVO_GLOBAL char *tab,
+                                                   const unsigned plane, const CVO_GLOBAL char *kept_w, const float *kept_a, const int packed,
+                                                   const unsigned ebase, const unsigned wcap, const unsigned n, const int lane, uint2 e, float w,
+                                                   double *acc)
+{
+    const float *Rt = hd.Rt, *tt = hd.tt;
+    for (unsigned off = lane; off < n; off += 64) {
+        if (off >= 64) { if (!PF) e = load8(kept_w, off); if (!packed) w = kept_a[off]; }
+        unsigned mi, mj;
+        float mw;
+        kept_unpack(packed, ebase, e, w, mi, mj, mw);
+        float4 xi = load_pos<false>(src.pos_a, mi * 16u);
+        float4 yj = load_pos<false>(src.pos_b, mj * 16u);
+        const float4 p0 = load_pos<true>(tab, mj * 16u);
+        const float4 p1 = load_pos<true>(tab + plane, mj * 16u);
+        const float4 p2 = load_pos<true>(tab + 2u * (size_t)plane, mj * 16u);
+        const float4 p3 = load_pos<false>(tab + 3u * (size_t)plane, mj * 16u);
+        if (PF) e = load8(kept_w, min(off + 64u, wcap - 1u));
+        if (src.tf_a) xi = apply_tf(Rt, tt, xi);
+        if (src.tf_b) yj = apply_tf(Rt, tt, yj);
+        if (!(mw > 0.0f)) continue;
+        StepPoint P;
+        P.bx[0] = p0.x; P.bx[1] = p0.y; P.bx[2] = p0.z; P.normxiz2 = p0.w;
+        P.gx[0] = p1.x; P.gx[1] = p1.y; P.gx[2] = p1.z; P.xz12 = p1.w;
+        P.dx[0] = p2.x; P.dx[1] = p2.y; P.dx[2] = p2.z; P.eps_c = p2.w;
+        P.ex[0] = p3.x; P.ex[1] = p3.y; P.ex[2] = p3.z; P.pad = 0.0f;
+        float beta, gamma, delta, epsil;
+        step_member_terms(kc, P, xi.x - yj.x, xi.y - yj.y, xi.z - yj.z, beta, gamma, delta, epsil);
+        step_tail(mw, beta, gamma, delta, epsil, acc);
     }
 }
 
@@ -916,6 +900,10 @@
         step_members2<PF>(src, hd, kc, xc, kept_w, a.kept_a + base, packed, ebase, wcap, n, lane, e, w, acc);
         if (false)
 #endif
+        if (hd.step_tab) {
+            step_members_table<PF>(src, hd, kc, pin_global<PIPE>(a.step_tab), pin_u32<PIPE>(a.step_tab_rows * 16u), kept_w, a.kept_a + base, packed,
+                                   ebase, wcap, n, lane, e, w, acc);
+        } else
         for (unsigned off = lane; off < n; off += 64) {
             if (off >= 64) { if (!PF) e = load8(kept_w, off); if (!packed) w = a.kept_a[base + off]; }
             uint2 e_next = e;
@@ -1119,7 +1107,7 @@
 
     ProcHead phd;
     phd.need_d2 = 0;
-    phd.narrow = 0; phd.rec_lim = PAD_BIG;
+    phd.narrow = 0; phd.rec_lim = PAD_BIG; phd.step_tab = 0;
     phd.Rt = hd->Rt; phd.tt = hd->t;
     double acc[NACC];
 #pragma unroll
@@ -1382,14 +1370,68 @@
     return *sh_fail == 0;
 }
 
+__device__ __forceinline__ bool step_table_wanted(const PostFlowArgs &a, const double members)
+{
+    return members >= 1.0 && members >= (double)a.tab_min * (double)a.tab_rows;
+}
+
+__device__ __forceinline__ void step_table_fill(const PostFlowArgs &a, double *sh, cvo_math::XiConsts *s_xi, double *s_red)
+{
+    const DevState *st = a.st;
+    if (a.check_done && (st->done != 0 || (a.prm.async_xy && st->stall))) return;
+    const unsigned ovf = (a.prm.async_xy ? 0u : st->ovf[0][LIST_XY]) | st->ovf[0][LIST_XX] | st->ovf[0][LIST_YY] | st->ovf[0][LIST_KEPT];
+    const KernConsts kc = st->kc;
+    float Rt[9], tt[3];
+#pragma unroll
+    for (int q = 0; q < 9; ++q) Rt[q] = st->Rt[q];
+#pragma unroll
+    for (int q = 0; q < 3; ++q) tt[q] = st->t[q];
+    if (a.tab_xi) {
+        block_reduce_partials<NACC_FLOW>(a.part_flow, a.nblk, sh, s_red);
+        if (threadIdx.x == 0) *s_xi = st->xi;
+        __syncthreads();
+    } else {
+        block_reduce_partials<NACC_FLOW>(a.part_flow, a.nblk, sh, s_red);
+    }
+    if (ovf != 0u || !step_table_wanted(a, s_red[8])) return;
+    if (!a.tab_xi) {
+        if (threadIdx.x < 64) {
+            float omega[3], v[3];
+            for (int q = 0; q < 3; ++q) { omega[q] = (float)s_red[q]; v[q] = (float)s_red[3 + q]; }
+            xi_consts_wave(s_xi, reinterpret_cast<float *>(sh), omega, v, (int)threadIdx.x);
+        }
+        __syncthreads();
+    }
+    const cvo_math::XiConsts xc = xi_uniform(*s_xi);
+    const unsigned rows = a.tab_rows, nb = gridDim.x - 1u;
+    for (unsigned j = (blockIdx.x - 1u) * BLOCK + threadIdx.x; j < rows; j += nb * BLOCK) {
+        float4 y = a.tab_pos[j];
+        if (a.tab_tf) y = apply_tf(Rt, tt, y);
+        step_point_store(a.step_tab, rows, j, step_point_terms(kc, xc, y.x, y.y, y.z));
+    }
+}
+
 __device__ __forceinline__ void post_flow_body(const PostFlowArgs &a)
 {
     __shared__ double sh[4 * NACC_MAX];
     __shared__ __attribute__((aligned(16))) DevHead s_st;
+    if (blockIdx.x != 0) {
+        if (a.step_tab) step_table_fill(a, sh, &s_st.xi, s_st.red);
+        return;
+    }
     state_head_to_lds(a.st, &s_st);
     DevHead *st = &s_st;
     if (a.check_done && (st->done != 0 || (a.prm.async_xy && st->stall))) return;
     const bool acvo = a.prm.mode == CVO_HIP_MODE_ACVO;
+    if (a.tab_xi) {
+        __shared__ double s_cnt[NACC_FLOW];
+        block_reduce_partials<NACC_FLOW>(a.part_flow, a.nblk, sh, s_cnt);
+        if (threadIdx.x == 0) {
+            const unsigned ovf = (a.prm.async_xy ? 0u : a.st->ovf[0][LIST_XY]) | a.st->ovf[0][LIST_XX] | a.st->ovf[0][LIST_YY] | a.st->ovf[0][LIST_KEPT];
+            a.st->step_tab_on = (a.step_tab && ovf == 0u && step_table_wanted(a, s_cnt[8])) ? 1 : 0;
+        }
+        return;
+    }
     if (a.flags & POST_REDUCE) {
         block_reduce_partials<NACC_FLOW>(a.part_flow, a.nblk, sh, st->red + RED_FLOW);
         if (acvo) {
@@ -1437,6 +1479,9 @@
             dl = num / (double)(nnz_xx + nnz_yy - 2 * nnz);
         }
         st->dl = dl;
+        const bool table = a.step_tab && !overflow && step_table_wanted(a, red[8]);
+        st->step_tab_on = table ? 1 : 0;
+        if (table) st->step_tab_passes += 1;
         if (!overflow && a.trace && st->k < a.trace_cap) {
             cvo_hip_trace &tr = a.trace[st->k];
             tr.k = st->k;
@@ -1853,7 +1898,9 @@
 {
     Grp<PostFlowArgs> g;
     for (int i = 0; i < n; ++i) g.a[i] = a[i];
-    hipLaunchKernelGGL(k_post_flow, dim3(1, 1, (unsigned)n), dim3(BLOCK), 0, s, g);
+    bool table = false;
+    for (int i = 0; i < n; ++i) table = table || a[i].step_tab != nullptr;
+    hipLaunchKernelGGL(k_post_flow, dim3(table ? 1u + STEP_TAB_BLOCKS : 1u, 1, (unsigned)n), dim3(BLOCK), 0, s, g);
 }
 
 void launch_post_step_group(const PostStepArgs *a, int n, hipStream_t s)
@@ -2055,6 +2102,7 @@
     hd.cand = nullptr; hd.cand_cnt = nullptr;
     hd.need_d2 = a.need_d2;
     hd.narrow = 0; hd.rec_lim = PAD_BIG;
+    hd.step_tab = 0;
     if (a.cand_b) {
         const int l = a.async_self == 2 ? 1 : 0;
         const int ck = MODE == PROC_FLOW ? (hd.second ? h->xy_ck[1] : h->xy_ck[0]) : (hd.second ? h->sf_ck[l][1] : h->sf_ck[l][0]);
@@ -3330,7 +3378,7 @@
         hd.cand = t ? pa.cand_b : pa.cand;
         hd.cand_cnt = t ? pa.cand_cnt_b : pa.cand_cnt;
         hd.need_d2 = 0;
-        hd.narrow = 0; hd.rec_lim = PAD_BIG;
+        hd.narrow = 0; hd.rec_lim = PAD_BIG; hd.step_tab = 0;
         process_body<PROC_FLOW, 0, true, false>(pa, blockIdx.x, scratch, hd);
     }
     __threadfence();
diff --git a/cvo-rgbd_amd/csrc/cvo_plan.cpp b/cvo-rgbd_amd/csrc/cvo_plan.cpp
--- a/cvo-rgbd_amd/csrc/cvo_plan.cpp
+++ b/cvo-rgbd_amd/csrc/cvo_plan.cpp
@@ -261,6 +261,13 @@
     a.need_d2 = (ctx->prm.mode == CVO_HIP_MODE_ACVO || !ctx->in_loop || ctx->cur_trace_cap > 0) ? 1 : 0;
     a.weight = ctx->prm.color_scale > 0.0f ? 1 : 0;
     a.kept_packed = kept_format(ctx, &a.kept_ebase);
+    if (mode == PROC_STEP) {
+        if (ctx->step_tab_armed && !ctx->merge_twist && pos_b == ctx->moving.pos) {
+            a.step_tab = (const float4 *)ctx->step_tab.p;
+            a.step_tab_rows = (unsigned)ctx->moving.np;
+        }
+        ctx->step_tab_armed = false;
+    }
     if ((mode == PROC_FLOW && list == LIST_XY) || (mode == PROC_SELF && (list == LIST_XX || list == LIST_YY))) {
         const bool no_cand = ctx->opt.no_cand;
         ctx->ck_nblk[list] = 0;
@@ -360,6 +367,40 @@
     return CVO_HIP_OK;
 }
 
+void arm_step_table(cvo_hip_ctx *ctx, PostFlowArgs &pa, bool xi_from_state)
+{
+    ctx->step_tab_armed = false;
+    if (ctx->opt.step_table_min < 0.0f || pa.comm || multi_rank(ctx) || ctx->merge_twist || ctx->moving.np <= 0) return;
+    if (!xi_from_state && pa.flags != (POST_REDUCE | POST_MATH)) return;
+    if (ensure_buf(ctx, ctx->step_tab, (size_t)ctx->moving.np * 4 * sizeof(float4)) != CVO_HIP_OK) {
+        (void)hipGetLastError();
+        ctx->err = "";
+        return;
+    }
+    pa.step_tab = (float4 *)ctx->step_tab.p;
+    pa.tab_rows = (unsigned)ctx->moving.np;
+    pa.tab_min = ctx->opt.step_table_min;
+    pa.tab_xi = xi_from_state ? 1 : 0;
+    const bool pre = pre_transform(ctx) && ctx->pos_bt.p;
+    pa.tab_pos = pre ? (const float4 *)ctx->pos_bt.p : ctx->moving.pos;
+    pa.tab_tf = pre ? 0 : 1;
+    ctx->step_tab_armed = true;
+}
+
+int enqueue_step_table(cvo_hip_ctx *ctx)
+{
+    PostFlowArgs pa{};
+    pa.st = ctx->st;
+    pa.prm = ctx->dprm;
+    pa.nblk = ctx->proc_blocks;
+    pa.part_flow = (const double *)ctx->part_flow.p;
+    arm_step_table(ctx, pa, true);
+    if (!pa.step_tab) return CVO_HIP_OK;
+    launch_post_flow(pa, ctx->stream);
+    HIP_TRY(ctx, hipGetLastError());
+    return CVO_HIP_OK;
+}
+
 void emit_post_flow(cvo_hip_ctx *ctx, const PostFlowArgs &pa)
 {
     if (ctx->rec) {
@@ -516,6 +557,7 @@
         }
     } else {
         pa.flags = POST_REDUCE | (do_math ? POST_MATH : 0);
+        arm_step_table(ctx, pa, false);
         emit_post_flow(ctx, pa);
     }
     HIP_TRY(ctx, hipGetLastError());
@@ -792,7 +834,7 @@
         if (q >= MAX_OPS) return false;
         const RecOp &op = ops[at];
         OpArgs &o = slot.op[q];
-        if (op.kind == RecOp::POST_FLOW) { o.pf = op.pf; plan.push_back(mk_launch(TK_POST_FLOW, q, 1, 1)); }
+        if (op.kind == RecOp::POST_FLOW) { o.pf = op.pf; plan.push_back(mk_launch(TK_POST_FLOW, q, 1u + STEP_TAB_BLOCKS, 1)); }
         else if (op.kind == RecOp::POST_STEP) {
             o.ps = op.ps;
             if (have_flow && flow.async_xy) o.ps.ck_nblk[LIST_XY] = 0;
@@ -873,7 +915,7 @@
                     gx = std::max(gx, (unsigned)op.p.nblk);
                 }
                 break;
-            case RecOp::POST_FLOW: o.pf = op.pf; kernel = TK_POST_FLOW; break;
+            case RecOp::POST_FLOW: o.pf = op.pf; kernel = TK_POST_FLOW; gx = 1u + STEP_TAB_BLOCKS; break;
             case RecOp::POST_STEP: o.ps = op.ps; kernel = TK_POST_STEP; break;
             }
         }
diff --git a/cvo-rgbd_amd/csrc/cvo_step.h b/cvo-rgbd_amd/csrc/cvo_step.h
--- /dev/null
+++ b/cvo-rgbd_amd/csrc/cvo_step.h
@@ -0,0 +1,100 @@
+#pragma once
+
+#include "cvo_device.h"
+
+namespace cvo_dev {
+
+CVO_HD double div6(double x)
+{
+    const double c = 0x1.5555555555555p-3;
+    const double q0 = x * c;
+    const double r = __builtin_fma(-6.0, q0, x);
+    return __builtin_fma(r, c, q0);
+}
+
+CVO_HD float mv_row(const float *m, float x, float y, float z)
+{
+    return (m[0] * x + m[1] * y) + m[2] * z;
+}
+
+struct StepPoint {
+    float bx[3], normxiz2;
+    float gx[3], xz12;
+    float dx[3], eps_c;
+    float ex[3], pad;
+};
+
+template <class XI>
+CVO_HD StepPoint step_point_terms(const KernConsts &kc, const XI &xc, const float yx, const float yy, const float yz)
+{
+    float xiz[3], xi2z[3], xi3z[3], xi4z[3];
+    xiz[0] = (xc.omega[1] * yz - xc.omega[2] * yy) + xc.v[0];
+    xiz[1] = (xc.omega[2] * yx - xc.omega[0] * yz) + xc.v[1];
+    xiz[2] = (xc.omega[0] * yy - xc.omega[1] * yx) + xc.v[2];
+#pragma unroll
+    for (int r = 0; r < 3; ++r) {
+        xi2z[r] = mv_row(xc.W2 + 3 * r, yx, yy, yz) + xc.u2[r];
+        xi3z[r] = mv_row(xc.W3 + 3 * r, yx, yy, yz) + xc.u3[r];
+        xi4z[r] = mv_row(xc.W4 + 3 * r, yx, yy, yz) + xc.u4[r];
+    }
+    StepPoint P;
+    P.normxiz2 = (xiz[0] * xiz[0] + xiz[1] * xiz[1]) + xiz[2] * xiz[2];
+    P.xz12 = -((xiz[0] * xi2z[0] + xiz[1] * xi2z[1]) + xiz[2] * xi2z[2]);
+    P.eps_c = ((xi2z[0] * xi2z[0] + xi2z[1] * xi2z[1]) + xi2z[2] * xi2z[2]) +
+              2 * ((xiz[0] * xi3z[0] + xiz[1] * xi3z[1]) + xiz[2] * xi3z[2]);
+    const float cb = kc.cb;
+#pragma unroll
+    for (int r = 0; r < 3; ++r) {
+        P.bx[r] = cb * xiz[r];
+        P.gx[r] = 2.0f * xi2z[r];
+        P.dx[r] = -xi3z[r];
+        P.ex[r] = 2.0f * xi4z[r];
+    }
+    P.pad = 0.0f;
+    return P;
+}
+
+CVO_HD void step_member_terms(const KernConsts &kc, const StepPoint &P, const float e0, const float e1, const float e2, float &beta,
+                              float &gamma, float &delta, float &epsil)
+{
+    const float cg = kc.cg, cd = kc.cd;
+    beta = (P.bx[0] * e0 + P.bx[1] * e1) + P.bx[2] * e2;
+    const float g_dot = (P.gx[0] * e0 + P.gx[1] * e1) + P.gx[2] * e2;
+    gamma = cg * (P.normxiz2 + g_dot);
+    const float d_dot = (P.dx[0] * e0 + P.dx[1] * e1) + P.dx[2] * e2;
+    delta = cd * (P.xz12 + d_dot);
+    const float e_dot = (P.ex[0] * e0 + P.ex[1] * e1) + P.ex[2] * e2;
+    epsil = cg * (P.eps_c + e_dot);
+}
+
+CVO_HD void step_tail(const float w, const float beta, const float gamma, const float delta, const float epsil, double *acc)
+{
+    const double A = (double)w;
+    const double b = (double)beta, g = (double)gamma;
+    acc[0] += (double)(w * beta);
+#ifdef CVO_STEP_TAIL_LITERAL
+    acc[1] += A * (g + (double)(beta * beta) / 2.0);
+    acc[2] += A * ((double)(delta + beta * gamma) + div6((double)(beta * beta * beta)));
+    acc[3] += A * ((((double)(epsil + beta * delta) + 0.5 * b * b * g) + 0.5 * g * g) +
+                   1 / 24.0 * b * b * b * b);
+#else
+    acc[1] = __builtin_fma(A, __builtin_fma((double)(beta * beta), 0.5, g), acc[1]);
+    acc[2] = __builtin_fma(A, __builtin_fma((double)(beta * beta * beta), 0x1.5555555555555p-3,
+                                            (double)(delta + beta * gamma)), acc[2]);
+    const double b2 = b * b, hg = 0.5 * g;
+    double t = __builtin_fma(b2, hg, (double)(epsil + beta * delta));
+    t = __builtin_fma(hg, g, t);
+    t = __builtin_fma(b2 * (1 / 24.0), b2, t);
+    acc[3] = __builtin_fma(A, t, acc[3]);
+#endif
+}
+
+CVO_HD void step_point_store(float4 *tab, const unsigned rows, const unsigned j, const StepPoint &P)
+{
+    tab[j] = make_float4(P.bx[0], P.bx[1], P.bx[2], P.normxiz2);
+    tab[rows + j] = make_float4(P.gx[0], P.gx[1], P.gx[2], P.xz12);
+    tab[2u * rows + j] = make_float4(P.dx[0], P.dx[1], P.dx[2], P.eps_c);
+    tab[3u * rows + j] = make_float4(P.ex[0], P.ex[1], P.ex[2], 0.0f);
+}
+
+}
```

Result: slower. 3716 registrations/s (-13.6%).
